# EndlessReform/fish-speech.rs

Hardware: AMD Instinct MI355X
Metric: codec tokens/sec (frames/s; 1 frame = 1 slow + 8 codebook tokens = 2048 PCM samples), Fish-1.5 batch=1 (higher is better)
Workload: dtype bf16

## Files before the change

### fish-speech.rs_amd/csrc/lm_engine.hip

```cpp
#include "lm_engine.h"

#include <algorithm>
#include <array>
#include <cmath>
#include <cstdlib>
#include <cstring>
#include <chrono>
#include <condition_variable>
#include <initializer_list>
#include <map>
#include <mutex>
#include <type_traits>
#include <vector>

#include <fcntl.h>
#include <sys/file.h>
#include <sys/stat.h>
#include <unistd.h>

#include "fs_common.h"
#include "fs_kv_pages.h"
#include "fs_prefill_plan.h"
#include "fs_synth.h"
#include "lm_kernels.h"
// ... 1573 lines not shown
            }
            launched += chunk;
            for (int b = 0; b < B_; ++b)
                if (slot_running(b)) {
                    sess_left_[b] -= chunk; sess_pos_[b] += chunk;
                    if (sess_left_[b] == 0 && !sess_.rows) {
                        static const int one = 1, zero = 0;
                        FS_HIP(hipMemcpyAsync(&state(b)->done, &one, sizeof(int), hipMemcpyHostToDevice, st_));
                        FS_HIP(hipMemcpyAsync(&state(b)->pos, &zero, sizeof(int), hipMemcpyHostToDevice, st_));
                        upload_row(b, st_, &sess_scratch_, 1);
                    }
                }
            FS_HIP(hipMemcpyAsync(sess_hs_.data(), state(0), sizeof(SeqState) * B_, hipMemcpyDeviceToHost, st_));
            tab_fetch_counts(hid_);
            tab_fetch_counts(sc_);
            FS_HIP(hipStreamSynchronize(st_));
            tab_take_counts(hid_);
            tab_take_counts(sc_);
            if (sess_.rows) rows_check_ctl(false);
            else check_rows_xchg();
        }
        FS_HIP(hipEventRecord(ev_[2], st_));
        FS_HIP(hipEventSynchronize(ev_[2]));
        float ms = 0;
        FS_HIP(hipEventElapsedTime(&ms, ev_[1], ev_[2]));
        stats_.decode_ms += ms;
        stats_.graph_launches += (uint64_t)launched;
        int act = 0;
        uint64_t frames = 0;
        for (int b = 0; b < B_; ++b) {
            if (slot_running(b) || slot_prefilling(b)) ++act;
            if (sess_left_[b] >= 0) frames += (uint64_t)sess_hs_[b].n_out;
        }
        stats_.frames = sess_released_frames_ + frames;
        if (n_active) *n_active = act;
    }
    void session_poll(int slot, uint32_t* codes_out, size_t cap, size_t* n_frames, int* done) override {
        use_device();
        require_live_slot(slot);
        const int C = a_.num_codebooks;
        const size_t nb = slot_prefilling(slot) ? 0 : (size_t)sess_hs_[slot].n_out;
        if (codes_out) {
            FS_REQUIRE(nb <= cap, "codes_out capacity too small for the generated frames");
            for (int c = 0; c < C; ++c)
                FS_HIP(hipMemcpyAsync(codes_out + (size_t)c * cap, d_out_.as<uint32_t>() + ((size_t)slot * C + c) * out_cap_, sizeof(uint32_t) * nb,
                                      hipMemcpyDeviceToHost, st_));
            FS_HIP(hipStreamSynchronize(st_));
        }
        if (n_frames) *n_frames = nb;
        if (done) *done = (!slot_prefilling(slot) && (sess_hs_[slot].done != 0 || sess_left_[slot] == 0)) ? 1 : 0;
    }
    void session_release(int slot) override {
        use_device();
        require_live_slot(slot);
        while (slot_prefilling(slot)) { flush_pending(); activate_pending(true); }
        sess_released_frames_ += (uint64_t)sess_hs_[slot].n_out;
        truncate(slot, 0);
        park_slot(slot, sess_.rows);
        tab_drop(hid_, slot);
        tab_drop(sc_, slot);
        sess_traced_[slot] = 0;
        sess_left_[slot] = kSlotFree;
    }
    void session_end() override {
        if (!sess_active_) return;
        use_device();
        if (!sess_flight_.empty()) (void)hipEventSynchronize(ev_pf_);
        std::string bad_book;
        try { pages_.check(); } catch (const std::exception& e) { bad_book = e.what(); }
        for (auto* q : {&sess_flight_, &sess_queue_})
            for (const PendingAdd& pa : *q) if (pa.tail >= 0) pages_.drop_hold(pa.tail);
        tab_end(hid_);
        tab_end(sc_);
        sess_flight_.clear(); sess_queue_.clear();
        pages_.end_session();
        std::fill(seq_len_.begin(), seq_len_.end(), 0);
        sess_prefixes_.clear();
        SampleCfg cfg = base_cfg();
        FS_HIP(hipMemcpyAsync(d_cfg_.p, &cfg, sizeof(cfg), hipMemcpyHostToDevice, st_));
        FS_HIP(hipStreamSynchronize(st_));
        sess_active_ = false;
        const bool rows = sess_.rows;
        sess_ = {};
        sess_released_frames_ = 0;
        if (rows) check_ctl({&d_rctl_s_, &d_rctl_f_}, nullptr, nullptr);
        if (sess_plock_.owns_lock()) sess_plock_.unlock();
        if (!bad_book.empty()) throw Error(bad_book);
    }

    void generate_batch_sequential(const uint32_t* prompts, const int* lens, int n, int max_new_tokens, const fs_sampling& s, uint64_t seed,
                                   uint32_t flags, uint32_t* codes_out, size_t cap, size_t* n_frames, uint8_t* is_audio) {
        if (legacy_) throw Error("generate_static_batch samples the slow token over the full vocabulary for Fish <= 1.4 (static_batch.rs:132-141); not implemented");
        const int C1 = a_.num_codebooks + 1;
        int Lmax = 0;
        for (int i = 0; i < n; ++i) { FS_REQUIRE(lens[i] >= 1, "empty prompt"); Lmax = std::max(Lmax, lens[i]); }
        fs_sampling sb = s;
        sb.repetition_penalty = 1.0f;
        size_t off = 0;
        std::vector<uint32_t> padded((size_t)C1 * Lmax);
        for (int i = 0; i < n; ++i) {
            left_pad(prompts + off, lens[i], Lmax, padded.data());
            off += (size_t)C1 * lens[i];
            clear_slow();
            batch_rows_ = n; batch_row_ = i;
            try {
                generate(padded.data(), Lmax, max_new_tokens, sb, seed, flags, codes_out + (size_t)i * a_.num_codebooks * cap, cap, &n_frames[i],
                         nullptr, nullptr, nullptr, 0, nullptr);
            } catch (...) { batch_rows_ = 0; batch_row_ = 0; throw; }
            batch_rows_ = 0; batch_row_ = 0;
            if (is_audio) {
                const SeqState* hs = reinterpret_cast<const SeqState*>(h_pin_);
                const bool first_not_audio = hs->frame == 1 && hs->cur[0] == t_.im_end_id;
                for (size_t f = 0; f < n_frames[i]; ++f) is_audio[(size_t)i * cap + f] = (f == 0 && first_not_audio) ? 0 : 1;
            }
        }
    }


    void generate_multi(const uint32_t* prompts, const int* lens, int n, const int* max_new_tokens, const fs_sampling* samplings,
                        const uint64_t* seeds, uint32_t flags, uint32_t* codes_out, size_t cap, size_t* n_frames) override {
        use_device();
        require_loaded();
        FS_REQUIRE(!sess_active_, "the handle is in session mode (fs_lm_session_end first)");
        FS_REQUIRE(n >= 1, "Must have at least one prompt");
        const int C = a_.num_codebooks, C1 = C + 1;
        std::vector<size_t> poff(n);
        {
            size_t off = 0;
            for (int i = 0; i < n; ++i) { FS_REQUIRE(lens[i] >= 1, "empty prompt"); FS_REQUIRE(max_new_tokens[i] >= 0, "negative max_new_tokens"); poff[i] = off; off += (size_t)C1 * lens[i]; }
        }
        bool rows_ok = rows_supported(n, samplings) && !(flags & FS_GEN_NO_PERSIST);
        const bool rows_sampled = samplings[0].temp != 0.0;
        std::unique_lock<PersistLock> plock;
        if (rows_ok) { plock = acquire_persist(device_); rows_ok = plock.owns_lock(); }
        if (!rows_ok) {
            if (plock.owns_lock()) plock.unlock();
            double pf = 0, dc = 0; uint64_t fr = 0, pt = 0, gl = 0;
            for (int i = 0; i < n; ++i) {
                clear_slow();
                generate(prompts + poff[i], lens[i], max_new_tokens[i], samplings[i], seeds[i], flags, codes_out + (size_t)i * C * cap, cap, &n_frames[i],
                         nullptr, nullptr, nullptr, 0, nullptr);
                pf += stats_.prefill_ms; dc += stats_.decode_ms; fr += stats_.frames; pt += stats_.prompt_tokens; gl += stats_.graph_launches;
            }
            stats_.prefill_ms = pf; stats_.decode_ms = dc; stats_.frames = fr; stats_.prompt_tokens = pt; stats_.graph_launches = gl;
            return;
        }
        const int R = n <= 2 ? 2 : (n <= 4 ? 4 : 8);
        ensure_rows(R);
        clear_slow();
        clear_fast();
        std::vector<long long> n_iter(n);
        long long max_iter = 0;
        for (int i = 0; i < n; ++i) {
            validate_tokens(prompts + poff[i], 0, 1, lens[i]);
            if (lens[i] > a_.max_seq_len) throw Error("prompt exceeds max_seq_len (dual_ar.rs:623-624)");
            n_iter[i] = iter_budget(max_new_tokens[i], lens[i]).n_iter;
            max_iter = std::max(max_iter, n_iter[i]);
            ensure_capacity(i, lens[i] + (int)n_iter[i] - 1);
        }
        std::vector<SampleCfg> cfgs(R);
        std::vector<int> budget(R, 0);
        for (int i = 0; i < R; ++i) {
            cfgs[i] = i < n ? make_cfg(samplings[i], flags) : base_cfg();
            if (i < n) budget[i] = (int)n_iter[i];
        }
        FS_HIP(hipMemcpyAsync(d_rcfg_.p, cfgs.data(), sizeof(SampleCfg) * R, hipMemcpyHostToDevice, st_));
        FS_HIP(hipMemcpyAsync(d_rbudget_.p, budget.data(), sizeof(int) * R, hipMemcpyHostToDevice, st_));
        float* nullp = nullptr;
        FS_HIP(hipMemcpyAsync(d_hid_slot_.p, &nullp, sizeof(nullp), hipMemcpyHostToDevice, st_));
        ensure_rows_capture(R);
        PersistFlagsGuard flags_guard{*this};
        stats_ = {};
        FS_HIP(hipEventRecord(ev_[0], st_));
        for (int i = 0; i < R; ++i) {
            SeqState ss = {};
            if (i >= n) { ss.done = 2; FS_HIP(hipMemcpyAsync(state(i), &ss, sizeof(ss), hipMemcpyHostToDevice, st_)); continue; }
            const int L = lens[i];
            ss.prompt_L = L;
            FS_HIP(hipMemcpyAsync(state(i), &ss, sizeof(ss), hipMemcpyHostToDevice, st_));
            FS_HIP(hipMemcpyAsync(main_.prompt.p, prompts + poff[i], sizeof(uint32_t) * C1 * L, hipMemcpyHostToDevice, st_));
            FS_HIP(hipMemcpyAsync(d_cfg_.p, &cfgs[i], sizeof(SampleCfg), hipMemcpyHostToDevice, st_));
            RngState rng;
            upload_rng(seeds[i], rng, d_rrng_.as<RngState>() + i, st_);
            launch_reppen_reset(rrp_.view(i), C, a_.codebook_size, st_);
            prefill_tokens(i, L - 1, false);
            LmKernels<WT>::embed(d_, tok_emb_, cb_emb_, C, a_.codebook_size, d_cfg_.as<SampleCfg>(), main_.prompt.as<uint32_t>(), state(i), x(i), st_);
            FS_HIP(hipStreamSynchronize(st_));
            seq_len_[i] = L - 1;
            stats_.prompt_tokens += (uint64_t)L;
        }
        use_persist_ = true; use_pslow_ = true; persist_sampled_ = rows_sampled;
        std::vector<SeqState> hs(R);
        auto all_done = [&]() {
            FS_HIP(hipMemcpyAsync(hs.data(), state(0), sizeof(SeqState) * R, hipMemcpyDeviceToHost, st_));
            FS_HIP(hipStreamSynchronize(st_));
            for (int i = 0; i < n; ++i) if (hs[i].done != 2) return false;
            return true;
        };
        int maxL = 0;
        for (int i = 0; i < n; ++i) maxL = std::max(maxL, lens[i]);
        const bool rows_fast = !getenv("FISHRT_ROWS_FAST_SINGLE");
        auto launch_frame = [&](long long it_) {
            set_bucket(maxL + (int)it_);
            RowsSlowArgs S = rows_slow_args(R);
            launch_rows_slow(S, R, st_);
            if (rows_fast) launch_rows_fast_groups(n, rows_sampled);
            else {
                static const int two = 2;
                for (int i = 0; i < n; ++i) {
                    if (it_ >= n_iter[i]) { if (it_ == n_iter[i]) FS_HIP(hipMemcpyAsync(&state(i)->done, &two, sizeof(int), hipMemcpyHostToDevice, st_)); continue; }
                    launch_fast_persist(persist_args(i), rows_sampled, st_);
                }
            }
        };
        launch_frame(0);
        FS_HIP(hipEventRecord(ev_[1], st_));
        long long it = 1;
        while (it < max_iter) {
            const long long end = std::min<long long>(max_iter, it + 32);
            for (; it < end; ++it) launch_frame(it);
            if (it < max_iter && all_done()) break;
        }
        if (!rows_fast) {
            static const int two = 2;
            for (int i = 0; i < n; ++i) FS_HIP(hipMemcpyAsync(&state(i)->done, &two, sizeof(int), hipMemcpyHostToDevice, st_));
        }
        FS_HIP(hipEventRecord(ev_[2], st_));
        FS_HIP(hipMemcpyAsync(hs.data(), state(0), sizeof(SeqState) * R, hipMemcpyDeviceToHost, st_));
        FS_HIP(hipStreamSynchronize(st_));
        use_persist_ = use_pslow_ = false;
        float ms01 = 0, ms12 = 0;
        FS_HIP(hipEventElapsedTime(&ms01, ev_[0], ev_[1]));
        FS_HIP(hipEventElapsedTime(&ms12, ev_[1], ev_[2]));
        stats_.prefill_ms = ms01; stats_.decode_ms = ms12; stats_.graph_launches = (uint64_t)it;
        stats_.kernels_per_frame = (uint64_t)(1 + (rows_fast ? (n + PR_FAST_ROWS - 1) / PR_FAST_ROWS : n));
        dump_rows_prof(R, it);
        rows_check_ctl(!rows_fast);
        stats_.frames = copy_out_rows(hs, n, codes_out, cap, n_frames);
    }

    bool rows_predicate(int n, const fs_sampling* ss, int ns, bool for_session, const char** why = nullptr) const {
        const char* w = nullptr;
        if (!(n >= 2 && n <= PR_MAX_ROWS && n <= B_)) w = "2 <= requests <= min(8, max_batch)";
        else if (!(loaded_ && pslow_ok_ && persist_ok_ && n_audio_ <= 2048)) w = "a loaded bf16 / fp8 handle with the Fish geometry on a 256-CU device";
        else if (getenv("FISHRT_NO_ROWS")) w = "FISHRT_NO_ROWS is set";
        else if (!rows_kv_span_ok(n <= 2 ? 2 : (n <= 4 ? 4 : 8))) w = "max_seq_len too long for the row kernels' attention slices at this row count";
        else if (for_session && legacy_) w = "row SESSIONS need the Fish 1.5 token layout (fs_lm_generate_multi serves Fish <= 1.4 handles)";
        else if (for_session && !(n == 2 || n == 4 || n == 8)) w = "row sessions need max_batch 2, 4 or 8";
        else {
            const bool sampled = ss[0].temp != 0.0;
            for (int i = 0; i < ns && !w; ++i) {
                if ((ss[i].temp != 0.0) != sampled) w = "every request greedy or every request sampled";
                else if (sampled && !fast_persist_samples((float)ss[i].temp, clamp_top_k(ss[i].top_k), a_.codebook_size)) w = "sampled requests with 0 < top_k <= 256";
            }
        }
        if (why) *why = w;
        return w == nullptr;
    }
    bool rows_supported(int n, const fs_sampling* samplings) override { return rows_predicate(n, samplings, n, false); }

  private:
    void use_device() { FS_HIP(hipSetDevice(device_)); }

    bool rows_kv_span_ok(int R) const {
        const int nslm = std::max(1, 16 / std::max(1, R));
        return ((a_.max_seq_len + nslm - 1) / nslm) / KV_PAGE + 2 <= 160;
    }
    void check_ctl(std::initializer_list<DevBuf*> bufs, const char* who, const char* bad_cfg_msg) {
        bool timeout = false, bad_cfg = false;
        for (DevBuf* cb : bufs) {
            if (!cb || !cb->p) continue;
            uint32_t ctl[4] = {0, 0, 0, 0};
            FS_HIP(hipMemcpy(ctl, cb->p, sizeof(ctl), hipMemcpyDeviceToHost));
            if (ctl[1] || ctl[2]) FS_HIP(hipMemset((uint32_t*)cb->p + 1, 0, 8));
            timeout |= ctl[1] != 0; bad_cfg |= ctl[2] != 0;
        }
        if (!who) return;
        if (timeout) {
            pslow_ok_ = persist_ok_ = false;
            throw Error(std::string(who) + ": a grid-wide wait timed out (are all 256 CUs available to this process?); "
                                           "the handle falls back to per-node launches for its next calls");
        }
        if (bad_cfg) throw Error(bad_cfg_msg);
    }
    void rows_check_ctl(bool include_b1_fast) {
        check_ctl({&d_rctl_s_, &d_rctl_f_, include_b1_fast ? &d_ctl_ : (DevBuf*)nullptr}, "request-row persistent kernels",
                  "request-row persistent kernels launched with a sampling configuration they were not built for");
    }
    void dump_persist_prof(int L) {
        if (!getenv("FISHRT_PERSIST_PROF")) return;
        unsigned long long pr[24];
        const double f = 0.01 / std::max<double>(1.0, (double)stats_.graph_launches - (double)L + 1);
        if (use_persist_) {
            FS_HIP(hipMemcpy(pr, d_ctl_.as<uint32_t>() + 16, sizeof(pr), hipMemcpyDeviceToHost));
            FS_HIP(hipMemset(d_ctl_.as<uint32_t>() + 16, 0, sizeof(pr)));
            fprintf(stderr, "persist prof (us/frame, workgroup 0; wait+work): preload %.1f  S1 %.1f+%.1f  S2 %.1f+%.1f  S3 %.1f+%.1f  S4 %.1f+%.1f  head %.1f+%.1f  decision %.1f+%.1f  tail %.1f | S3 split: gemv+reduce %.1f barrier %.1f epilogue %.1f\n",
                    pr[0] * f, pr[9] * f, pr[1] * f, pr[10] * f, pr[2] * f, pr[11] * f, pr[3] * f, pr[12] * f, pr[4] * f, pr[13] * f, pr[5] * f, pr[14] * f, pr[6] * f, pr[7] * f, pr[8] * f, pr[15] * f, pr[3] * f);
            fprintf(stderr, "persist boundaries (us/frame, workgroup 0): slow kernel's finish -> fast kernel's entry %.2f (%llu frames)  entry -> first stage timer (state, slow-token decision) %.2f  last timer -> finish %.2f\n",
                    pr[20] ? pr[17] * 0.01 / (double)pr[20] : 0.0, pr[20], pr[18] * f, pr[19] * f);
        }
        if (use_pslow_) {
            FS_HIP(hipMemcpy(pr, d_sctl_.as<uint32_t>() + 16, sizeof(pr), hipMemcpyDeviceToHost));
            FS_HIP(hipMemset(d_sctl_.as<uint32_t>() + 16, 0, sizeof(pr)));
            fprintf(stderr, "slow persist prof (us/frame, workgroup %d; wait+work): S1 %.1f+%.1f  S2 %.1f+%.1f  S3 %.1f+%.1f  S4 %.1f+%.1f  S5 %.1f+%.1f  head %.1f+%.1f\n",
                    getenv("FISHRT_PERSIST_PROF_WG") ? atoi(getenv("FISHRT_PERSIST_PROF_WG")) : 0, pr[9] * f, pr[1] * f, pr[10] * f, pr[2] * f, pr[11] * f, pr[3] * f,
                    pr[12] * f, pr[4] * f, pr[13] * f, pr[5] * f, pr[14] * f, pr[6] * f);
            fprintf(stderr, "slow persist boundaries (us/frame): fast kernel's finish -> slow kernel's entry %.2f (%llu frames)  entry -> first stage timer (state, first loads) %.2f  last timer -> finish %.2f\n",
                    pr[20] ? pr[17] * 0.01 / (double)pr[20] : 0.0, pr[20], pr[18] * f, pr[19] * f);
        }
    }
    void dump_rows_prof(int R, long long frames) {
        if (!getenv("FISHRT_PERSIST_PROF")) return;
        unsigned long long pr[16];
        const double f = 0.01 / std::max<double>(1.0, (double)frames);
        FS_HIP(hipMemcpy(pr, d_rctl_s_.as<uint32_t>() + 16, sizeof(pr), hipMemcpyDeviceToHost));
        FS_HIP(hipMemset(d_rctl_s_.as<uint32_t>() + 16, 0, sizeof(pr)));
        fprintf(stderr, "rows slow prof R=%d (us/frame, workgroup 0): S1 %.1f  S2 %.1f  S3 sweep %.1f + %.1f  S4 sweep %.1f gemm %.1f barrier %.1f publish %.1f  S5 sweep+gemm %.1f barrier %.1f publish %.1f  head %.1f\n",
                R, pr[1] * f, pr[2] * f, pr[8] * f, pr[3] * f, pr[9] * f, pr[10] * f, pr[11] * f, pr[4] * f, pr[12] * f, pr[13] * f, pr[5] * f, pr[6] * f);
        FS_HIP(hipMemcpy(pr, d_rctl_f_.as<uint32_t>() + 16, sizeof(pr), hipMemcpyDeviceToHost));
        FS_HIP(hipMemset(d_rctl_f_.as<uint32_t>() + 16, 0, sizeof(pr)));
        fprintf(stderr, "rows fast prof (us/frame summed over the fast launches, workgroup 0; wait+work): preload %.1f  S1 %.1f+%.1f  S2 %.1f+%.1f  S3 %.1f+%.1f  S4 %.1f+%.1f  head %.1f+%.1f  decision %.1f+%.1f (rows' logits -> argmax / draw %.1f, pick -> next input %.1f)  tail %.1f\n",
                pr[0] * f, pr[9] * f, pr[1] * f, pr[10] * f, pr[2] * f, pr[11] * f, (pr[3] + pr[8]) * f, pr[12] * f, pr[4] * f, pr[13] * f, pr[5] * f, pr[14] * f, (pr[6] + pr[15]) * f, pr[15] * f, pr[6] * f, pr[7] * f);
    }
    void upload_rng(uint64_t seed, RngState& host, RngState* dst, hipStream_t st) {
        host = RngState{};
        seed_from_u64(seed, host.key);
        FS_HIP(hipMemcpyAsync(dst, &host, sizeof(host), hipMemcpyHostToDevice, st));
    }
    void left_pad(const uint32_t* prompt, int L, int Lmax, uint32_t* out) const {
        const int C1 = a_.num_codebooks + 1, pad = Lmax - L;
        for (int r = 0; r < C1; ++r) {
            for (int j = 0; j < pad; ++j) out[(size_t)r * Lmax + j] = r == 0 ? t_.im_end_id : 0u;
            std::memcpy(&out[(size_t)r * Lmax + pad], prompt + (size_t)r * L, sizeof(uint32_t) * L);
        }
    }
    uint64_t copy_out_rows(const std::vector<SeqState>& hs, int n, uint32_t* codes_out, size_t cap, size_t* n_frames) {
        const int C = a_.num_codebooks;
        std::vector<uint32_t> tmp((size_t)n * C * out_cap_);
        FS_HIP(hipMemcpy(tmp.data(), d_out_.p, sizeof(uint32_t) * tmp.size(), hipMemcpyDeviceToHost));
        uint64_t total = 0;
        for (int i = 0; i < n; ++i) {
            const size_t nb = (size_t)hs[i].n_out;
            FS_REQUIRE(nb <= cap, "codes_out capacity too small for the generated frames");
            for (int c = 0; c < C; ++c)
                std::memcpy(codes_out + ((size_t)i * C + c) * cap, tmp.data() + ((size_t)i * C + c) * out_cap_, sizeof(uint32_t) * nb);
            n_frames[i] = nb;
            total += nb;
            seq_len_[i] = hs[i].pos;
        }
        return total;
    }
    void launch_rows_fast_groups(int top, bool sampled) {
        for (int r0 = 0; r0 < top; r0 += PR_FAST_ROWS) {
            const int left = std::min(PR_FAST_ROWS, top - r0), Rf = left >= 3 ? 4 : left;
            launch_rows_fast(rows_fast_args(r0, Rf), Rf, sampled, st_);
        }
    }
    struct PersistFlagsGuard {
        LM& lm;
        ~PersistFlagsGuard() { lm.use_persist_ = lm.use_pslow_ = false; }
    };
    void require_loaded() { FS_REQUIRE(loaded_, "weights not loaded: call fs_lm_load_safetensors or fs_lm_load_synthetic first"); }

    static int clamp_top_k(uint64_t top_k) { return (int)std::min<uint64_t>(top_k, 1u << 30); }
    SampleCfg make_cfg(const fs_sampling& s, uint32_t flags) const {
        SampleCfg c = base_cfg();
        c.temp = (float)s.temp; c.top_p = (float)s.top_p; c.top_p64 = s.top_p;
        c.top_k = clamp_top_k(s.top_k);
        c.rep_pen = s.repetition_penalty; c.ignore_eos = (flags & FS_GEN_IGNORE_EOS) ? 1 : 0;
        return c;
    }
    struct Budget { long long n_iter; bool clamped; };
    Budget iter_budget(long long max_new, long long L_total, long long n_cached = 0) const {
        Budget b{1 + std::max<long long>(0, max_new - L_total + 1), false};
        const long long room = (long long)a_.max_seq_len - (n_cached + L_total) + 1;
        if (b.n_iter > room) { b.n_iter = room; b.clamped = true; }
        FS_REQUIRE(b.n_iter <= out_cap_, "generation longer than the output staging buffer");
        return b;
    }
    SampleCfg base_cfg() const {
        SampleCfg c = {};
        c.temp = 0.f; c.top_p = 1.f; c.top_k = 0; c.rep_pen = 1.f; c.ignore_eos = 0;
        c.im_end_id = t_.im_end_id;
        c.audio_base = legacy_ ? t_.im_end_id : t_.semantic_start_id - 1;
        c.sem_lo = t_.semantic_start_id;
        c.sem_hi = t_.has_semantic_end ? t_.semantic_end_id : t_.semantic_start_id;
        c.legacy = legacy_ ? 1 : 0;
        c.pad_id = t_.pad_id;
        return c;
    }

    void validate_tokens(const uint32_t* toks, size_t, int B, int L) {
        const int C1 = a_.num_codebooks + 1;
        for (int b = 0; b < B; ++b)
            for (int r = 0; r < C1; ++r)
                for (int l = 0; l < L; ++l) {
                    const uint32_t v = toks[((size_t)b * C1 + r) * L + l];
                    if (r == 0) { if (v >= (uint32_t)a_.vocab_size) throw Error("token id out of vocabulary (index_select out of range)"); }
                    else if (v >= (uint32_t)a_.codebook_size) throw Error("codebook id out of range (index_select out of range)");
                }
    }

    void plan_tensors() {
        size_t off = 0;
        auto align = [&](size_t v) { return (v + 255) & ~(size_t)255; };
        auto mat = [&](const std::string& name, int64_t rows, int64_t cols, int mul, int roff, std::pair<size_t, size_t> at) {
            tensors_.push_back({name, rows, cols, false, false, at.first, at.second, mul, roff, 0.f, 0.02});
        };
        auto emb = [&](const std::string& name, int64_t rows, int64_t cols) {
            size_t at = off;
            off = align(off + (size_t)rows * cols * sizeof(KT));
            tensors_.push_back({name, rows, cols, false, true, at, 0, 1, 0, 0.f, 0.02});
            return at;
        };
        auto slab = [&](int64_t rows, int64_t cols) {
            std::pair<size_t, size_t> at{off, 0};
            off = align(off + (size_t)rows * cols * sizeof(WT));
            if (kFp8) { at.second = off; off = align(off + (size_t)rows * sizeof(float)); }
            return at;
        };
        auto vec = [&](const std::string& name, int64_t n) {
            size_t at = off;
            off = align(off + (size_t)n * sizeof(float));
            tensors_.push_back({name, 1, n, true, false, at, 0, 1, 0, 1.0f, 0.1});
            return at;
        };
        const int64_t D = a_.dim, I = a_.intermediate_size, V = a_.vocab_size;
        const int64_t QKV = (int64_t)(a_.n_head + 2 * a_.n_local_heads) * a_.head_dim;
        o_tok_emb_ = emb("embeddings.weight", V, D);
        o_cb_emb_ = emb("codebook_embeddings.weight", (int64_t)a_.codebook_size * a_.num_codebooks, D);
        auto blocks = [&](int n, const std::string& pre, std::vector<std::array<size_t, 10>>& offs) {
            for (int l = 0; l < n; ++l) {
                const std::string p = pre + std::to_string(l) + ".";
                std::array<size_t, 10> o;
                auto s0 = slab(QKV, D); mat(p + "attention.wqkv.weight", QKV, D, 1, 0, s0);
                auto s1 = slab(D, D); mat(p + "attention.wo.weight", D, D, 1, 0, s1);
                auto s2 = slab(2 * I, D);
                mat(p + "feed_forward.w1.weight", I, D, 2, 0, s2);
                mat(p + "feed_forward.w3.weight", I, D, 2, 1, s2);
                auto s3 = slab(D, I); mat(p + "feed_forward.w2.weight", D, I, 1, 0, s3);
                o[0] = s0.first; o[1] = s1.first; o[2] = s2.first; o[3] = s3.first;
                o[4] = vec(p + "ffn_norm.weight", D);
                o[5] = vec(p + "attention_norm.weight", D);
                o[6] = s0.second; o[7] = s1.second; o[8] = s2.second; o[9] = s3.second;
                offs.push_back(o);
            }
        };
        blocks(a_.n_layer, "layers.", o_slow_);
        o_norm_ = vec("norm.weight", D);
        if (a_.tie_word_embeddings && !kFp8) o_out_ = {o_tok_emb_, 0};
        else { o_out_ = slab(V, D); mat(a_.tie_word_embeddings ? "embeddings.weight" : "output.weight", V, D, 1, 0, o_out_); }
        o_fast_emb_ = emb("fast_embeddings.weight", a_.codebook_size, D);
        blocks(a_.n_fast_layer, "fast_layers.", o_fast_);
        o_fast_norm_ = vec("fast_norm.weight", D);
        o_fast_out_ = slab(a_.codebook_size, D); mat("fast_output.weight", a_.codebook_size, D, 1, 0, o_fast_out_);
        arena_bytes_ = off;
    }

    void alloc_runtime() {
        arena_.alloc(arena_bytes_);
        uint8_t* base = arena_.as<uint8_t>();
        auto lw = [&](const std::array<size_t, 10>& o) {
            LayerW w;
            w.wqkv = base + o[0]; w.wo = base + o[1]; w.w13 = base + o[2]; w.w2 = base + o[3];
            w.ffn_norm = (const float*)(base + o[4]); w.attn_norm = (const float*)(base + o[5]);
            if (kFp8) {
                w.s_qkv = (const float*)(base + o[6]); w.s_o = (const float*)(base + o[7]);
                w.s_13 = (const float*)(base + o[8]); w.s_2 = (const float*)(base + o[9]);
            }
            return w;
        };
        for (auto& o : o_slow_) slow_.push_back(lw(o));
        for (auto& o : o_fast_) { fast_.push_back(lw(o)); fast_.back().cache_resident = getenv("FISHRT_FAST_NT") == nullptr; }
        tok_emb_ = base + o_tok_emb_; cb_emb_ = base + o_cb_emb_; fast_emb_ = base + o_fast_emb_;
        out_w_ = base + o_out_.first; fast_out_w_ = base + o_fast_out_.first;
        if (kFp8) { out_s_ = (const float*)(base + o_out_.second); fast_out_s_ = (const float*)(base + o_fast_out_.second); }
        norm_w_ = (const float*)(base + o_norm_); fast_norm_w_ = (const float*)(base + o_fast_norm_);
        const int half = a_.head_dim / 2, n_elem = a_.dim / a_.n_head;
        std::vector<float> ct((size_t)a_.max_seq_len * half), sn((size_t)a_.max_seq_len * half), theta(half);
        for (int j = 0; j < half; ++j) theta[j] = 1.f / std::pow(a_.rope_base, (float)(2 * j) / (float)n_elem);
        for (int p = 0; p < a_.max_seq_len; ++p)
            for (int j = 0; j < half; ++j) {
                const float ang = (float)p * theta[j];
                ct[(size_t)p * half + j] = std::cos(ang);
                sn[(size_t)p * half + j] = std::sin(ang);
            }
        d_cos_.alloc(ct.size() * 4); d_sin_.alloc(sn.size() * 4);
        FS_HIP(hipMemcpy(d_cos_.p, ct.data(), ct.size() * 4, hipMemcpyHostToDevice));
        FS_HIP(hipMemcpy(d_sin_.p, sn.data(), sn.size() * 4, hipMemcpyHostToDevice));
        n_chunks_ = (a_.max_seq_len + AttnKernels<WT>::chunk() - 1) / AttnKernels<WT>::chunk();
        FS_REQUIRE(n_chunks_ <= 128, "max_seq_len too large for the attention chunking (128 chunks)");
        max_pages_ = std::max((a_.max_seq_len + KV_PAGE - 1) / KV_PAGE, n_chunks_ * AttnKernels<WT>::chunk() / KV_PAGE);
        n_pages_ = max_pages_ * B_;
        page_elems_ = (size_t)a_.n_local_heads * KV_PAGE * a_.head_dim;
        kv_pool_.alloc((size_t)a_.n_layer * 2 * n_pages_ * page_elems_ * sizeof(KT));
        FS_HIP(hipMemset(kv_pool_.p, 0, kv_pool_.n));
        d_page_table_.alloc(sizeof(int) * (size_t)std::max(2 * B_ + 1, PR_MAX_ROWS) * max_pages_);
        FS_HIP(hipMemset(d_page_table_.p, 0, d_page_table_.n));
        pages_.init(n_pages_, B_, KV_PAGE, a_.max_seq_len);
        seq_len_.assign(B_, 0);
        fast_len_.assign(B_, 0);
        fast_pool_.alloc((size_t)std::max(1, a_.n_fast_layer) * 2 * B_ * page_elems_ * sizeof(KT));
        FS_HIP(hipMemset(fast_pool_.p, 0, fast_pool_.n));
        d_zero_table_.alloc(sizeof(int) * 4);
        FS_HIP(hipMemset(d_zero_table_.p, 0, d_zero_table_.n));
        d_x_.alloc(sizeof(float) * (size_t)std::max(B_, PR_MAX_ROWS) * a_.dim);
        d_xf_.alloc(sizeof(float) * (size_t)std::max(B_, PR_MAX_ROWS) * a_.dim);
        FS_HIP(hipMemset(d_x_.p, 0, d_x_.n));
        d_q_.alloc(sizeof(float) * a_.dim);
        d_part_.alloc(sizeof(float) * (size_t)a_.n_head * n_chunks_ * (a_.head_dim + 2));
        FS_HIP(hipMemset(d_part_.p, 0, d_part_.n));
        d_act_.alloc(sizeof(float) * a_.intermediate_size);
        d_logits_slow_.alloc(sizeof(float) * a_.vocab_size);
        d_logits_fast_.alloc(sizeof(float) * a_.codebook_size);
        d_hid_slot_.alloc(sizeof(float*));
        FS_HIP(hipMemset(d_hid_slot_.p, 0, sizeof(float*)));
        d_state_.alloc(sizeof(SeqState) * (std::max(B_, PR_MAX_ROWS) + 1));
        FS_HIP(hipMemset(d_state_.p, 0, d_state_.n));
        d_cfg_.alloc(sizeof(SampleCfg));
        SampleCfg c = base_cfg();
        FS_HIP(hipMemcpy(d_cfg_.p, &c, sizeof(c), hipMemcpyHostToDevice));
        d_rng_.alloc(sizeof(RngState));
        main_.prompt.alloc(sizeof(uint32_t) * (size_t)(a_.num_codebooks + 1) * a_.max_seq_len);
        out_cap_ = a_.max_seq_len + 8;
        d_out_.alloc(sizeof(uint32_t) * (size_t)B_ * a_.num_codebooks * out_cap_);
        rp_.alloc(1, a_.num_codebooks, a_.codebook_size);
        FS_HIP(hipHostMalloc(&h_pin_, 4096, hipHostMallocDefault));
    }

    const void* slow_head_w() {
        if (!legacy_ && !generic_) return (const uint8_t*)out_w_ + (size_t)t_.im_end_id * a_.dim * sizeof(WT);
        if (!d_legacy_head_.p) d_legacy_head_.alloc(gathered_head_bytes() + sizeof(float) * n_audio_ + 256);
        return d_legacy_head_.p;
    }
    size_t gathered_head_bytes() const { return ((sizeof(WT) * (size_t)n_audio_ * a_.dim) + 15) & ~(size_t)15; }
    const float* slow_head_s() {
        if (!kFp8) return nullptr;
        if (!legacy_ && !generic_) return out_s_ + t_.im_end_id;
        slow_head_w();
        return (const float*)(d_legacy_head_.as<uint8_t>() + gathered_head_bytes());
    }
    void refresh_legacy_head() {
        if (generic_) {
            const size_t row = sizeof(WT) * (size_t)a_.dim;
            uint8_t* dst = (uint8_t*)const_cast<void*>(slow_head_w());
            FS_HIP(hipMemcpyAsync(dst, (const uint8_t*)out_w_ + t_.im_end_id * row, row, hipMemcpyDeviceToDevice, st_));
            FS_HIP(hipMemcpyAsync(dst + row, (const uint8_t*)out_w_ + t_.semantic_start_id * row, row * (n_audio_ - 1), hipMemcpyDeviceToDevice, st_));
            if (kFp8) {
                float* ds = const_cast<float*>(slow_head_s());
                FS_HIP(hipMemcpyAsync(ds, out_s_ + t_.im_end_id, sizeof(float), hipMemcpyDeviceToDevice, st_));
                FS_HIP(hipMemcpyAsync(ds + 1, out_s_ + t_.semantic_start_id, sizeof(float) * (n_audio_ - 1), hipMemcpyDeviceToDevice, st_));
            }
            FS_HIP(hipStreamSynchronize(st_));
            return;
        }
        if (!legacy_) return;
        launch_gather_rows<WT>(out_w_, a_.dim, t_.pad_id, t_.im_end_id, const_cast<void*>(slow_head_w()), st_);
        if (kFp8) launch_gather_rows<float>(out_s_, 1, t_.pad_id, t_.im_end_id, const_cast<float*>(slow_head_s()), st_);
        FS_HIP(hipStreamSynchronize(st_));
    }
    SeqState* state(int b) { return d_state_.as<SeqState>() + b; }
    float* x(int b) { return d_x_.as<float>() + (size_t)b * a_.dim; }
    float* xf(int b) { return d_xf_.as<float>() + (size_t)b * a_.dim; }
    KVView slow_kv(int layer, int b) {
        KVView v;
        KT* base = kv_pool_.as<KT>() + (size_t)layer * 2 * n_pages_ * page_elems_;
        v.k = base; v.v = base + (size_t)n_pages_ * page_elems_;
        v.page_table = d_page_table_.as<int>() + (size_t)b * max_pages_;
        return v;
    }
    KVView fast_kv(int layer, int b) {
        KVView v;
        KT* base = fast_pool_.as<KT>() + ((size_t)layer * 2 * B_) * page_elems_;
        v.k = base + (size_t)b * page_elems_;
        v.v = base + ((size_t)B_ + b) * page_elems_;
        v.page_table = d_zero_table_.as<int>();
        return v;
    }

    void ensure_capacity(int b, int n_tokens) {
        if (!pages_.grow(b, n_tokens)) return;
        upload_row(b, st_, pages_.of(b));
        FS_HIP(hipStreamSynchronize(st_));
    }
    void truncate(int b, int pos) {
        pages_.truncate(b, pos);
        seq_len_[b] = pos;
    }
    void upload_row(int row, hipStream_t st, const int* ids, size_t n) {
        FS_HIP(hipMemcpyAsync(d_page_table_.as<int>() + (size_t)row * max_pages_, ids, sizeof(int) * n, hipMemcpyHostToDevice, st));
    }
    void upload_row(int row, hipStream_t st, const std::vector<int>& ids) { upload_row(row, st, ids.data(), ids.size()); }

    void prefill_tokens(int b, int n, bool use_graph) {
        if (n <= 0) return;
        if (RowKernels<WT>::has_mfma_prefill() && n > 1 && a_.dim % 128 == 0 && a_.intermediate_size % 128 == 0) {
            ensure_prefill_buffers();
            const int M = launch_seq_pass(main_, state(b), b, seq_len_[b], n);
            FS_HIP(hipMemcpyAsync(x(b), main_.x.as<float>() + (size_t)(M - 1) * a_.dim, sizeof(float) * a_.dim, hipMemcpyDeviceToDevice, st_));
            return;
        }
        for (int l = 0; l < n; ++l) {
            set_bucket(seq_len_[b] + l + 1);
            if (use_graph && b == 0) { use_graphs_for_bucket(); FS_HIP(hipGraphLaunch(g_step_, st_)); continue; }
            LmKernels<WT>::embed(d_, tok_emb_, cb_emb_, a_.num_codebooks, a_.codebook_size, d_cfg_.as<SampleCfg>(),
                                 main_.prompt.as<uint32_t>(), state(b), x(b), st_);
            enqueue_slow_layers(b);
            launch_advance(state(b), st_);
        }
    }
    int launch_seq_pass(PrefillLane& ln, SeqState* st, int kv_row, int start, int n) {
        RowsCtx c = ln.ctx(st, 1, 0);
        int M = 0;
        for (int done = 0; done < n; done += M) {
            M = std::min(a_.head_dim == 64 ? kRowsCap : kPartRows, n - done);
            c.nc_launch = chunk_bucket(start + done + M);
            RowKernels<WT>::prefill_embed(d_, tok_emb_, cb_emb_, a_.num_codebooks, a_.codebook_size, d_cfg_.as<SampleCfg>(),
                                         ln.prompt.as<uint32_t>(), st, M, ln.x.as<float>(), ln.st);
            for (int l = 0; l < a_.n_layer; ++l) RowKernels<WT>::rows_layer(d_, M, c, slow_[l], slow_kv(l, kv_row), l == 0, ln.st);
            RowKernels<WT>::rows_finish(d_, M, c, nullptr, ln.st);
            launch_advance_n(st, M, ln.st);
        }
        return M;
    }
    void launch_group_pass(PrefillLane& ln, const uint32_t* prompts, int S, int Lp, size_t pstride, SeqState* st, int kv_row,
                           const SeqState* seq_states, int nc_launch) {
        RowsCtx c = ln.ctx(st, 1, max_pages_);
        c.seq_rows = Lp;
        c.nc_launch = nc_launch;
        c.seq_states = seq_states;
        const int M = S * Lp;
        RowKernels<WT>::prefill_embed(d_, tok_emb_, cb_emb_, a_.num_codebooks, a_.codebook_size, d_cfg_.as<SampleCfg>(), prompts, st, M,
                                     ln.x.as<float>(), ln.st, Lp, pstride);
        for (int l = 0; l < a_.n_layer; ++l) RowKernels<WT>::rows_layer(d_, M, c, slow_[l], slow_kv(l, kv_row), l == 0, ln.st);
    }
    void ensure_prefill_buffers() {
        if (main_.x.p) return;
        const int I = a_.intermediate_size;
        down_split_ = I % 1024 == 0 ? I / 1024 : (I % 256 == 0 ? I / 256 : I / 128);
        main_.ensure(a_, down_split_, n_chunks_, d_cos_.as<float>(), d_sin_.as<float>());
    }
    void check_rows_xchg() {
        if (!d_epoch_.p) return;
        uint32_t e[2] = {0, 0};
        FS_HIP(hipMemcpy(e, d_epoch_.p, sizeof(e), hipMemcpyDeviceToHost));
        if (e[1] != 0) {
            const uint32_t z = 0;
            FS_HIP(hipMemcpy(d_epoch_.as<uint32_t>() + 1, &z, sizeof(z), hipMemcpyHostToDevice));
            fold_off_ = true;
            drop_batch_graphs();
            throw Error("static-batch decode: " + std::to_string(e[1]) + " split-K exchange waits timed out (a down projection's blocks were not co-resident); "
                        "this handle falls back to the slab path for its next calls");
        }
    }
    void ensure_batch_buffers() {
        if (d_xfrows_.p) return;
        ld_slow_ = ((n_audio_ + 63) / 64) * 64;
        d_xfrows_.alloc(sizeof(float) * kRows * a_.dim);
        d_lrows_.alloc(sizeof(float) * kRows * ld_slow_);
        d_lfast_.alloc(sizeof(float) * kRows * a_.codebook_size);
        std::vector<SeqState> fs(8);
        for (int i = 0; i < 8; ++i) { fs[i] = SeqState{}; fs[i].pos = i; }
        d_fast_state_.alloc(sizeof(SeqState) * 8);
        FS_HIP(hipMemcpy(d_fast_state_.p, fs.data(), sizeof(SeqState) * 8, hipMemcpyHostToDevice));
        std::vector<int> tb(B_);
        for (int i = 0; i < B_; ++i) tb[i] = i;
        d_rwords_.alloc(sizeof(uint32_t) * 16 * kRows);
        d_xchg_.alloc(rows_xchg_bytes(a_.dim));
        FS_HIP(hipMemset(d_xchg_.p, 0, d_xchg_.n));
        d_epoch_.alloc(sizeof(uint32_t) * 2);
        const uint32_t e0[2] = {1u, 0u};
        FS_HIP(hipMemcpy(d_epoch_.p, e0, sizeof(e0), hipMemcpyHostToDevice));
        d_fast_table_.alloc(sizeof(int) * B_);
        FS_HIP(hipMemcpy(d_fast_table_.p, tb.data(), sizeof(int) * B_, hipMemcpyHostToDevice));
        hid_.dev.alloc(sizeof(HidSlot) * B_);
        FS_HIP(hipMemset(hid_.dev.p, 0, hid_.dev.n));
        sc_.dev.alloc(sizeof(ScoreSlot) * B_);
        FS_HIP(hipMemset(sc_.dev.p, 0, sc_.dev.n));
    }
    void enqueue_batch_frame(int B) {
        const int C = a_.num_codebooks;
        RowsCtx cs = main_.ctx(state(0), sess_active_ ? -1 : 0, max_pages_);
        cs.nc_launch = nc_launch_;
        cs.xchg = d_xchg_.p; cs.epoch = d_epoch_.as<uint32_t>();
        const bool fold = !fold_off_ && RowKernels<WT>::rows_fold_ok(d_, B, cs) && a_.n_layer <= 64 && a_.n_fast_layer <= 8 && C <= 32;
        cs.fold = fold;
        for (int l = 0; l < a_.n_layer; ++l, cs.node_id = (uint32_t)l)
            RowKernels<WT>::rows_layer(d_, B, cs, slow_[l], slow_kv(l, 0), l == 0, st_, fold ? (l + 1 < a_.n_layer ? slow_[l + 1].attn_norm : norm_w_) : nullptr);
        if (!fold) RowKernels<WT>::rows_finish(d_, B, cs, norm_w_, st_);
        RowKernels<WT>::rows_head(d_, B, cs, slow_head_w(), slow_head_s(), n_audio_, d_lrows_.as<float>(), ld_slow_, st_, fold);
        if (sess_active_) launch_hidden_rows(hid_.dev.as<HidSlot>(), state(0), cs.X, a_.dim, B, st_);
        const bool slots = sess_.slots;
        const uint32_t* words = rows_par_ ? d_rwords_.as<uint32_t>() : nullptr;
        if (rows_par_) SampleKernels<WT>::rows_rng_words(d_rng_.as<RngState>(), B, C + 1, state(0), d_rwords_.as<uint32_t>(), st_);
        const bool capt = cap_frames_ > 0 && d_rcap_.p && d_rcap_.n >= sizeof(float) * (size_t)B * cap_frames_ * 9 * 2048;
        if (capt) launch_cap_rows_logits(d_lrows_.as<float>(), ld_slow_, n_audio_, state(0), d_cfg_.as<SampleCfg>(), B, d_rcap_.as<float>(), cap_frames_, 0, st_);
        const float* prep_g = fold && a_.dim <= 1024 ? fast_[0].attn_norm : nullptr;
        const bool score = slots && sess_.score;
        const bool trace = score && sess_.trace;
        float* stash = trace ? d_trace_.as<float>() : nullptr;
        const int alts = score ? sess_.alts : 0;
        if (score) launch_score_slots(sc_.dev.as<ScoreSlot>(), state(0), d_scfg_.as<SampleCfg>(), d_lrows_.as<float>(), ld_slow_, n_audio_, 0, C, B, st_, stash, alts);
        if (slots)
            SampleKernels<WT>::sample_slow_slots(d_, d_lrows_.as<float>(), ld_slow_, n_audio_, d_scfg_.as<SampleCfg>(), d_srng_.as<SlotRng>(), B, state(0),
                                                 cs.X, d_xfrows_.as<float>(), st_, prep_g, cs.A, fold ? d_epoch_.as<uint32_t>() : nullptr,
                                                 capt ? d_rcap_.as<float>() : nullptr, cap_frames_, sess_.wide);
        else
        SampleKernels<WT>::sample_slow_rows(d_, d_lrows_.as<float>(), ld_slow_, n_audio_, d_cfg_.as<SampleCfg>(), d_rng_.as<RngState>(), B,
                                            C + 1, state(0), cs.X, d_xfrows_.as<float>(), st_, words, prep_g, cs.A, fold ? d_epoch_.as<uint32_t>() : nullptr);
        const bool qkv0_on = fold && d_qkv0_.p && !getenv("FISHRT_ROWS_NO_QKV0") && a_.codebook_size == 1024;
        auto fast_ctx = [&](int cbi) {
            RowsCtx cf = cs;
            cf.X = d_xfrows_.as<float>();
            cf.state = d_fast_state_.as<SeqState>() + cbi;
            cf.pos_step = 0;
            cf.pt_stride = 1;
            cf.nc_launch = 1;
            cf.small_attn = a_.num_codebooks <= 8;
            cf.identity_pages = true;
            cf.attn_t1 = cbi == 0;
            if (qkv0_on && AttnKernels<WT>::rows_qkv0_ok(d_, cf)) { cf.qkv0_tbl = d_qkv0_.as<float>(); cf.row_states = state(0); cf.code_slot = cbi; }
            return cf;
        };
        RowsCtx cf = fast_ctx(0);
        cf.first_prepped = prep_g != nullptr;
        for (int cbi = 0; cbi < C; ++cbi) {
            for (int l = 0; l < a_.n_fast_layer; ++l) {
                KVView kv;
                KT* base = fast_pool_.as<KT>() + ((size_t)l * 2 * B_) * page_elems_;
                kv.k = base; kv.v = base + (size_t)B_ * page_elems_; kv.page_table = d_fast_table_.as<int>();
                cf.node_id = 64u + (uint32_t)cbi * 8u + (uint32_t)l;
                RowKernels<WT>::rows_layer(d_, B, cf, fast_[l], kv, l == 0, st_, fold ? (l + 1 < a_.n_fast_layer ? fast_[l + 1].attn_norm : fast_norm_w_) : nullptr);
            }
            if (!fold) RowKernels<WT>::rows_finish(d_, B, cf, fast_norm_w_, st_);
            RowKernels<WT>::rows_head(d_, B, cf, fast_out_w_, kFp8 ? fast_out_s_ : nullptr, a_.codebook_size, d_lfast_.as<float>(), a_.codebook_size, st_, fold);
            if (capt) launch_cap_rows_logits(d_lfast_.as<float>(), a_.codebook_size, a_.codebook_size, state(0), d_cfg_.as<SampleCfg>(), B, d_rcap_.as<float>(),
                                             cap_frames_, 1 + cbi, st_);
            RowsCtx nf = fast_ctx(cbi + 1);
            const float* prep_f = nf.qkv0_tbl ? nullptr : prep_g;
            nf.first_prepped = prep_f != nullptr;
            if (score) launch_score_slots(sc_.dev.as<ScoreSlot>(), state(0), d_scfg_.as<SampleCfg>(), d_lfast_.as<float>(), a_.codebook_size, a_.codebook_size,
                                          1 + cbi, C, B, st_, stash, alts);
            if (slots) {
                RepPenState rp0 = srp_.view(0);
                SampleKernels<WT>::sample_fast_slots(d_, d_lfast_.as<float>(), cbi, C, a_.codebook_size, d_scfg_.as<SampleCfg>(), d_srng_.as<SlotRng>(), rp0,
                                                     B, state(0), fast_emb_, d_xfrows_.as<float>(), tok_emb_, cb_emb_, cs.X, d_out_.as<uint32_t>(), out_cap_,
                                                     st_, prep_f, cs.A, sess_.wide);
            } else
            SampleKernels<WT>::sample_fast_rows(d_, d_lfast_.as<float>(), cbi, C, a_.codebook_size, d_cfg_.as<SampleCfg>(),
                                                d_rng_.as<RngState>(), B, state(0), fast_emb_, d_xfrows_.as<float>(), tok_emb_, cb_emb_,
                                                cs.X, d_out_.as<uint32_t>(), out_cap_, st_, words, prep_f, cs.A);
            cf = nf;
        }
        if (trace) launch_trace_commit(sc_.dev.as<ScoreSlot>(), state(0), d_scfg_.as<SampleCfg>(), stash, n_audio_, a_.codebook_size, C, B, st_, alts);
        if (capt) launch_cap_rows_picks(state(0), d_cfg_.as<SampleCfg>(), B, d_rcap_.as<float>(), cap_frames_, C, st_);
    }
    void ensure_rows_capture(int B) {
        if (!cap_frames_) return;
        FS_REQUIRE((size_t)B * cap_frames_ <= 4096, "decision capture on the row path: rows x frames limited to 4096 (302 MB)");
        d_rcap_.alloc(sizeof(float) * (size_t)B * cap_frames_ * 9 * 2048);
        FS_HIP(hipMemsetAsync(d_rcap_.p, 0, d_rcap_.n, st_));
    }
    void drop_batch_graphs() {
        for (auto& kv : batch_graphs_) if (kv.second) (void)hipGraphExecDestroy(kv.second);
        batch_graphs_.clear();
    }
    void destroy_graphs() {
        for (auto& kv : graphs_)
            for (hipGraphExec_t g : {kv.second.first, kv.second.second}) if (g) (void)hipGraphExecDestroy(g);
        graphs_.clear();
        for (auto& kv : multi_graphs_) if (kv.second) (void)hipGraphExecDestroy(kv.second);
        multi_graphs_.clear();
        g_frame_ = g_step_ = nullptr;
        drop_batch_graphs();
    }
    hipGraphExec_t batch_graph(int B) {
        const long long key = (sess_active_ ? 1 << 24 : 0) + (rows_par_ ? 1 << 25 : 0) + (sess_.slots ? 1 << 26 : 0) + (sess_.slots && sess_.wide ? 1 << 27 : 0) +
                              (sess_.slots && sess_.score ? 1 << 28 : 0) + (sess_.slots && sess_.score && sess_.trace ? 1 << 29 : 0) + B * 1024 + nc_launch_ +
                              ((long long)(sess_.slots && sess_.score ? sess_.alts : 0) << 32);
        auto it = batch_graphs_.find(key);
        if (it != batch_graphs_.end()) return it->second;
        {
            RowsCtx cs = main_.ctx(state(0), 0, max_pages_);
            cs.xchg = d_xchg_.p; cs.epoch = d_epoch_.as<uint32_t>();
            (void)RowKernels<WT>::rows_fold_ok(d_, B, cs);
        }
        hipGraph_t g = nullptr;
        hipGraphExec_t ge = nullptr;
        FS_HIP(hipStreamBeginCapture(st_, hipStreamCaptureModeThreadLocal));
        enqueue_batch_frame(B);
        FS_HIP(hipStreamEndCapture(st_, &g));
        FS_HIP(hipGraphInstantiate(&ge, g, nullptr, nullptr, 0));
        FS_HIP(hipGraphDestroy(g));
        batch_graphs_[key] = ge;
        return ge;
    }

    static constexpr int kNapsFast[6] = {16, 16, 16, 16, 16, 16}, kNapsSlow[6] = {20, 16, 6, 36, 36, 12};
    static constexpr int kNapsFastSampled[6] = {12, 16, 12, 20, 12, 16}, kNapsSlowFp8[6] = {20, 4, 28, 24, 24, 0};
    static constexpr bool kSlowStreamNt = true, kSlowStreamNtFp8 = true;
    static void set_naps(int (&naps)[6], const char* env, const int (&dflt)[6]) {
        for (int i = 0; i < 6; ++i) naps[i] = dflt[i];
        if (const char* v = getenv(env)) {
            int i = 0;
            for (const char* p = v; *p && i < 6; ++i) { naps[i] = atoi(p); while (*p && *p != ',') ++p; if (*p == ',') ++p; }
        }
    }
    void pack_persist() {
        persist_ok_ = false;
        if (d_qkv0_.p) { destroy_graphs(); d_qkv0_.free(); }
        if constexpr (std::is_same<WT, bf16_t>::value || std::is_same<WT, fp8_t>::value) {
            constexpr bool FP8 = std::is_same<WT, fp8_t>::value;
            if (getenv("FISHRT_NO_PERSIST")) return;
            if (!fast_persist_supported(d_, a_.n_fast_layer, a_.num_codebooks, a_.codebook_size)) return;
            hipDeviceProp_t prop;
            FS_HIP(hipGetDeviceProperties(&prop, device_));
            if (prop.multiProcessorCount < PF_BLOCKS) return;
            if (!d_pack_.p) {
                d_pack_.alloc(fast_persist_pack_bytes());
                d_edges_.alloc(fast_persist_edge_bytes());
                FS_HIP(hipMemset(d_edges_.p, 0, d_edges_.n));
                d_ctl_.alloc(320);
                FS_HIP(hipMemset(d_ctl_.p, 0, d_ctl_.n));
                if (FP8) d_fscl_.alloc(sizeof(float) * (size_t)PF_BLOCKS * PF_SCL);
            }
            launch_fast_persist_pack(fast_.data(), fast_out_w_, d_pack_.p, st_, FP8, fast_out_s_, d_fscl_.as<float>());
            if (!getenv("FISHRT_FAST_NO_QKV0")) {
                d_qkv0_.alloc(fast_persist_qkv0_bytes());
                launch_fast_persist_qkv0_table(d_pack_.p, FP8 ? d_fscl_.as<float>() : nullptr, fast_[0].attn_norm, fast_emb_, d_.eps, d_qkv0_.as<float>(), st_);
            }
            FS_HIP(hipStreamSynchronize(st_));
            persist_ok_ = true;
            pslow_ok_ = false;
            if (getenv("FISHRT_NO_PERSIST_SLOW") || n_audio_ > 8 * PF_BLOCKS) return;
            if (const char* c = getenv("FISHRT_SLOW_STREAM"))
                FS_REQUIRE(strcmp(c, "default") == 0 || strcmp(c, "nt") == 0, "FISHRT_SLOW_STREAM must be 'default' or 'nt'");
            if (!d_spack_.p) {
                d_spack_.alloc(slow_persist_pack_bytes(a_.n_layer, FP8));
                d_hpack_.alloc((size_t)PF_BLOCKS * PS_HEAD_IMAGE);
                if (FP8) d_sscl_.alloc(sizeof(float) * slow_persist_scale_floats(a_.n_layer));
                d_snorms_.alloc(sizeof(float) * (size_t)(2 * a_.n_layer + 1) * a_.dim);
                d_sedges_.alloc(slow_persist_edge_bytes());
                FS_HIP(hipMemset(d_sedges_.p, 0, d_sedges_.n));
                d_sctl_.alloc(320);
                FS_HIP(hipMemset(d_sctl_.p, 0, d_sctl_.n));
            }
            std::vector<const float*> np;
            for (int l = 0; l < a_.n_layer; ++l) { np.push_back(slow_[l].attn_norm); np.push_back(slow_[l].ffn_norm); }
            np.push_back(norm_w_);
            if (FP8) launch_slow_persist_pack_fp8(slow_.data(), a_.n_layer, slow_head_w(), slow_head_s(), n_audio_, np.data(), d_spack_.p, d_hpack_.p,
                                                  d_sscl_.as<float>(), d_snorms_.as<float>(), st_);
            else launch_slow_persist_pack(slow_.data(), a_.n_layer, slow_head_w(), n_audio_, np.data(), d_spack_.p, d_hpack_.p, d_snorms_.as<float>(), st_);
            FS_HIP(hipStreamSynchronize(st_));
            pslow_ok_ = true;
        }
    }
    SlowPersistArgs pslow_args() {
        SlowPersistArgs A = {};
        A.wpack = d_spack_.p; A.hpack = d_hpack_.p; A.norms = d_snorms_.as<float>();
        A.scales = d_sscl_.p ? d_sscl_.as<float>() : nullptr;
        A.hscales = d_sscl_.p ? d_sscl_.as<float>() + (size_t)a_.n_layer * PF_BLOCKS * 48 : nullptr;
        A.n_layer = a_.n_layer; A.n_head_rows = n_audio_;
        A.cos_t = d_cos_.as<float>(); A.sin_t = d_sin_.as<float>(); A.eps = d_.eps;
        A.x = x(0); A.logits = d_logits_slow_.as<float>(); A.state = state(0);
        A.kv_pool = kv_pool_.p; A.layer_half = (size_t)n_pages_ * page_elems_;
        A.page_table = d_page_table_.as<int>();
        A.n_sl = std::min(nc_launch_, nc_launch_ > 32 ? 16 : 8);
        if (const char* c = getenv("FISHRT_NSL_MAX")) A.n_sl = std::max(1, std::min(A.n_sl, atoi(c)));
        if (const char* c = getenv("FISHRT_NSL_MIN")) A.n_sl = std::min(16, std::max(A.n_sl, atoi(c)));
        while (A.n_sl & (A.n_sl - 1)) A.n_sl &= A.n_sl - 1;
        A.edges = d_sedges_.as<unsigned long long>();
        A.ctl = d_sctl_.as<uint32_t>();
        A.prof = getenv("FISHRT_PERSIST_PROF") ? reinterpret_cast<unsigned long long*>(d_sctl_.as<uint32_t>() + 16) : nullptr;
        A.peer_stamps = (A.prof && d_ctl_.p) ? reinterpret_cast<const unsigned long long*>(d_ctl_.as<uint32_t>() + 16) + 16 : nullptr;
        set_naps(A.naps, "FISHRT_NAPS_SLOW", kFp8 ? kNapsSlowFp8 : kNapsSlow);
        A.prof_wg = getenv("FISHRT_PERSIST_PROF_WG") ? atoi(getenv("FISHRT_PERSIST_PROF_WG")) : 0;
        A.l2_touch = (getenv("FISHRT_SLOW_EARLY") ? atoi(getenv("FISHRT_SLOW_EARLY")) : (kFp8 ? 1 : 9)) & 15;
        bool stream_nt = kFp8 ? kSlowStreamNtFp8 : kSlowStreamNt;
        if (const char* c = getenv("FISHRT_SLOW_STREAM")) stream_nt = strcmp(c, "nt") == 0;
        if (stream_nt) A.l2_touch |= PS_STREAM_NT;
        return A;
    }
    bool fold_slow_sampler() const { return use_persist_ && n_audio_ <= 2048; }
    FastPersistArgs persist_args() {
        FastPersistArgs A = {};
        A.wpack = d_pack_.p;
        A.scales = d_fscl_.p ? d_fscl_.as<float>() : nullptr;
        for (int l = 0; l < PF_LAYERS; ++l) { A.norms[2 * l] = fast_[l].attn_norm; A.norms[2 * l + 1] = fast_[l].ffn_norm; }
        A.norms[2 * PF_LAYERS] = fast_norm_w_;
        A.fast_emb = fast_emb_; A.tok_emb = tok_emb_; A.cb_emb = cb_emb_;
        A.qkv0_tbl = d_qkv0_.p ? d_qkv0_.as<float>() : nullptr;
        A.cos_t = d_cos_.as<float>(); A.sin_t = d_sin_.as<float>();
        A.eps = d_.eps;
        const bool fold = fold_slow_sampler();
        A.xf = fold ? x(0) : xf(0); A.x = x(0);
        A.slow_logits = fold ? d_logits_slow_.as<float>() : nullptr; A.n_slow = n_audio_; A.hid_slot = d_hid_slot_.as<float*>();
        A.cap = d_cap_.as<float>(); A.cap_frames = cap_frames_;
        A.state = state(0); A.cfg = d_cfg_.as<SampleCfg>(); A.rp = rp_.view(0); A.rng = d_rng_.as<RngState>();
        A.out_codes = d_out_.as<uint32_t>(); A.out_cap = out_cap_;
        A.edges = d_edges_.as<unsigned long long>();
        A.ctl = d_ctl_.as<uint32_t>();
        A.prof = getenv("FISHRT_PERSIST_PROF") ? reinterpret_cast<unsigned long long*>(d_ctl_.as<uint32_t>() + 16) : nullptr;
        A.peer_stamps = (A.prof && d_sctl_.p) ? reinterpret_cast<const unsigned long long*>(d_sctl_.as<uint32_t>() + 16) + 16 : nullptr;
        set_naps(A.naps, "FISHRT_NAPS_FAST", persist_sampled_ ? kNapsFastSampled : kNapsFast);
        return A;
    }


    void ensure_rows(int R) {
        if constexpr (std::is_same<WT, bf16_t>::value || kFp8) {
            if (!d_rimg_.p) {
                d_rimg_.alloc(slow_persist_pack_bytes(a_.n_layer, false));
                d_rhimg_.alloc((size_t)PF_BLOCKS * PS_HEAD_IMAGE);
                if constexpr (kFp8) launch_rows_pack_fp8(slow_.data(), a_.n_layer, slow_head_w(), n_audio_, d_rimg_.p, d_rhimg_.p, st_);
                else launch_rows_pack(slow_.data(), a_.n_layer, slow_head_w(), n_audio_, d_rimg_.p, d_rhimg_.p, st_);
                if constexpr (!kFp8) {
                    const size_t n1 = (size_t)a_.n_layer * PF_BLOCKS * 48 + (size_t)PF_BLOCKS * 8 + (size_t)PF_BLOCKS * PF_SCL;
                    std::vector<float> ones(n1, 1.0f);
                    d_rones_.alloc(n1 * sizeof(float));
                    FS_HIP(hipMemcpyAsync(d_rones_.p, ones.data(), n1 * sizeof(float), hipMemcpyHostToDevice, st_));
                    FS_HIP(hipStreamSynchronize(st_));
                }
                d_rpairs_.alloc((size_t)PF_BLOCKS * 40 * PF_THREADS * 4);
                launch_rows_pack_rowpairs(d_pack_.p, d_rpairs_.p, st_);
                d_redges_s_.alloc(rows_slow_edge_bytes(PR_MAX_ROWS));
                FS_HIP(hipMemsetAsync(d_redges_s_.p, 0, d_redges_s_.n, st_));
                d_redges_f_.alloc(rows_fast_edge_bytes(PR_FAST_ROWS));
                FS_HIP(hipMemsetAsync(d_redges_f_.p, 0, d_redges_f_.n, st_));
                d_rctl_s_.alloc(256); d_rctl_f_.alloc(256);
                FS_HIP(hipMemsetAsync(d_rctl_s_.p, 0, 256, st_));
                FS_HIP(hipMemsetAsync(d_rctl_f_.p, 0, 256, st_));
                d_rlogits_.alloc(sizeof(float) * PR_MAX_ROWS * PR_LD);
                d_rcfg_.alloc(sizeof(SampleCfg) * PR_MAX_ROWS);
                d_rrng_.alloc(sizeof(RngState) * PR_MAX_ROWS);
                d_rbudget_.alloc(sizeof(int) * PR_MAX_ROWS);
                rrp_.alloc(PR_MAX_ROWS, a_.num_codebooks, a_.codebook_size);
                FS_HIP(hipStreamSynchronize(st_));
            }
            (void)R;
        } else {
            throw Error("request rows need a bf16 or fp8 handle");
        }
    }
    static constexpr int kNapsRowsSlow[6] = {28, 4, 8, 40, 24, 28}, kNapsRowsFast[6] = {20, 16, 16, 16, 20, 20};
    RowsSlowArgs rows_slow_args(int R) {
        RowsSlowArgs A = {};
        A.wimg = d_rimg_.p; A.himg = d_rhimg_.p; A.norms = d_snorms_.as<float>();
        const float* sc0 = kFp8 ? d_sscl_.as<float>() : d_rones_.as<float>();
        A.scales = sc0;
        A.hscales = sc0 + (size_t)a_.n_layer * PF_BLOCKS * 48;
        A.n_layer = a_.n_layer; A.n_head_rows = n_audio_;
        A.cos_t = d_cos_.as<float>(); A.sin_t = d_sin_.as<float>(); A.eps = d_.eps;
        A.x = x(0); A.logits = d_rlogits_.as<float>(); A.state = state(0);
        A.kv_pool = kv_pool_.p; A.layer_half = (size_t)n_pages_ * page_elems_;
        A.page_table = d_page_table_.as<int>(); A.pt_stride = max_pages_;
        A.n_sl = std::max(1, std::min(nc_launch_, 16 / R));
        if (const char* c = getenv("FISHRT_ROWS_NSL_MAX")) A.n_sl = std::max(1, std::min(A.n_sl, atoi(c)));
        A.edges = d_redges_s_.as<unsigned long long>();
        A.ctl = d_rctl_s_.as<uint32_t>();
        A.prof = getenv("FISHRT_PERSIST_PROF") ? reinterpret_cast<unsigned long long*>(d_rctl_s_.as<uint32_t>() + 16) : nullptr;
        set_naps(A.naps, "FISHRT_NAPS_ROWS_SLOW", kNapsRowsSlow);
        return A;
    }
    RowsFastArgs rows_fast_args(int r0, int Rf) {
        RowsFastArgs A = {};
        (void)Rf;
        A.wpack = d_pack_.p; A.rowpairs = d_rpairs_.as<uint32_t>();
        A.scales = kFp8 ? d_fscl_.as<float>() : d_rones_.as<float>() + (size_t)a_.n_layer * PF_BLOCKS * 48 + (size_t)PF_BLOCKS * 8;
        for (int l = 0; l < PF_LAYERS; ++l) { A.norms[2 * l] = fast_[l].attn_norm; A.norms[2 * l + 1] = fast_[l].ffn_norm; }
        A.norms[2 * PF_LAYERS] = fast_norm_w_;
        A.fast_emb = fast_emb_; A.tok_emb = tok_emb_; A.cb_emb = cb_emb_;
        A.qkv0_tbl = (d_qkv0_.p && !getenv("FISHRT_ROWS_FAST_NO_QKV0")) ? d_qkv0_.as<float>() : nullptr;
        A.cos_t = d_cos_.as<float>(); A.sin_t = d_sin_.as<float>(); A.eps = d_.eps;
        A.xf = x(r0); A.x = x(r0);
        A.slow_logits = d_rlogits_.as<float>() + (size_t)r0 * PR_LD; A.n_slow = n_audio_;
        A.cap = cap_frames_ ? d_rcap_.as<float>() + (size_t)r0 * cap_frames_ * 9 * 2048 : nullptr; A.cap_frames = cap_frames_;
        A.state = state(r0); A.cfg = d_rcfg_.as<SampleCfg>() + r0; A.budget = d_rbudget_.as<int>() + r0; A.rng = d_rrng_.as<RngState>() + r0;
        const RepPenState rp = rrp_.view(r0);
        A.rp_mask = rp.mask; A.rp_ring = rp.ring; A.rp_meta = rp.ring_meta;
        A.out_codes = d_out_.as<uint32_t>() + (size_t)r0 * a_.num_codebooks * out_cap_; A.out_cap = out_cap_;
        A.edges = d_redges_f_.as<unsigned long long>();
        A.ctl = d_rctl_f_.as<uint32_t>();
        A.prof = getenv("FISHRT_PERSIST_PROF") ? reinterpret_cast<unsigned long long*>(d_rctl_f_.as<uint32_t>() + 16) : nullptr;
        set_naps(A.naps, "FISHRT_NAPS_ROWS_FAST", kNapsRowsFast);
        A.nap_draw = getenv("FISHRT_NAP_ROWS_DRAW") ? atoi(getenv("FISHRT_NAP_ROWS_DRAW")) : 16;
        return A;
    }
    FastPersistArgs persist_args(int i) {
        FastPersistArgs A = persist_args();
        A.xf = x(i); A.x = x(i);
        A.slow_logits = d_rlogits_.as<float>() + (size_t)i * PR_LD;
        A.cap = cap_frames_ ? d_rcap_.as<float>() + (size_t)i * cap_frames_ * 9 * 2048 : nullptr;
        A.state = state(i); A.cfg = d_rcfg_.as<SampleCfg>() + i; A.rp = rrp_.view(i); A.rng = d_rrng_.as<RngState>() + i;
        A.out_codes = d_out_.as<uint32_t>() + (size_t)i * a_.num_codebooks * out_cap_;
        return A;
    }

    void enqueue_slow_layers(int b) {
        for (int l = 0; l < a_.n_layer; ++l) {
            const LayerW& w = slow_[l];
            KVView kv = slow_kv(l, b);
            LmKernels<WT>::qkv(d_, x(b), w, d_cos_.as<float>(), d_sin_.as<float>(), state(b), 0, 0, d_q_.as<float>(), kv, st_);
            AttnKernels<WT>::decode(d_, d_q_.as<float>(), kv, state(b), d_part_.as<float>(), n_chunks_, nc_launch_, st_);
            LmKernels<WT>::wo(d_, d_part_.as<float>(), n_chunks_, nc_launch_, state(b), nullptr, kv, 0, w, x(b), st_);
            LmKernels<WT>::ffn_up(d_, x(b), w, d_act_.as<float>(), st_);
            LmKernels<WT>::ffn_down(d_, d_act_.as<float>(), w, x(b), st_);
        }
    }
    void enqueue_fast_layers(int b, int kv_pos, int rope_pos) {
        for (int l = 0; l < a_.n_fast_layer; ++l) {
            const LayerW& w = fast_[l];
            KVView kv = fast_kv(l, b);
            LmKernels<WT>::qkv(d_, xf(b), w, d_cos_.as<float>(), d_sin_.as<float>(), nullptr, kv_pos, rope_pos, d_q_.as<float>(), kv, st_);
            LmKernels<WT>::wo(d_, nullptr, 0, 0, nullptr, d_q_.as<float>(), kv, kv_pos + 1, w, xf(b), st_);
            LmKernels<WT>::ffn_up(d_, xf(b), w, d_act_.as<float>(), st_);
            LmKernels<WT>::ffn_down(d_, d_act_.as<float>(), w, xf(b), st_);
        }
    }

    int chunk_bucket(int T) const {
        const int need = (T + AttnKernels<WT>::chunk() - 1) / AttnKernels<WT>::chunk();
        int b = 1;
        while (b < need) b <<= 1;
        return std::min(b, n_chunks_);
    }
    void set_bucket(int T) { nc_launch_ = chunk_bucket(T); }
    void use_graphs_for_bucket() {
        const int key = nc_launch_ * 8 + (use_persist_ && persist_sampled_ ? 4 : 0) + (use_persist_ ? 2 : 0) + (use_pslow_ ? 1 : 0);
        auto it = graphs_.find(key);
        if (it == graphs_.end()) {
            g_frame_ = nullptr; g_step_ = nullptr;
            build_graphs();
            graphs_[key] = {g_frame_, g_step_};
        } else {
            g_frame_ = it->second.first; g_step_ = it->second.second;
        }
    }
    void build_graphs() {
        if (g_frame_) return;
        FS_REQUIRE(a_.num_codebooks <= 8, "the fused fast-decoder attention holds at most 8 positions");
        const int C = a_.num_codebooks;
        hipGraph_t g = nullptr;
        FS_HIP(hipStreamBeginCapture(st_, hipStreamCaptureModeThreadLocal));
        LmKernels<WT>::embed(d_, tok_emb_, cb_emb_, C, a_.codebook_size, d_cfg_.as<SampleCfg>(), main_.prompt.as<uint32_t>(), state(0), x(0), st_);
        enqueue_slow_layers(0);
        launch_advance(state(0), st_);
        FS_HIP(hipStreamEndCapture(st_, &g));
        FS_HIP(hipGraphInstantiate(&g_step_, g, nullptr, nullptr, 0));
        FS_HIP(hipGraphDestroy(g));
        FS_HIP(hipStreamBeginCapture(st_, hipStreamCaptureModeThreadLocal));
        if (use_pslow_) launch_slow_persist(pslow_args(), st_);
        else {
        enqueue_slow_layers(0);
        LmKernels<WT>::head(d_, x(0), norm_w_, slow_head_w(), slow_head_s(), n_audio_, d_logits_slow_.as<float>(), st_);
        }
        if (!fold_slow_sampler())
            SampleKernels<WT>::sample_slow(d_, d_logits_slow_.as<float>(), n_audio_, d_cfg_.as<SampleCfg>(), d_rng_.as<RngState>(), state(0),
                                           x(0), xf(0), st_, d_hid_slot_.as<float*>());
        if (use_persist_) launch_fast_persist(persist_args(), persist_sampled_, st_);
        else
        for (int cbi = 0; cbi < C; ++cbi) {
            enqueue_fast_layers(0, cbi, cbi);
            LmKernels<WT>::head(d_, xf(0), fast_norm_w_, fast_out_w_, fast_out_s_, a_.codebook_size, d_logits_fast_.as<float>(), st_);
            SampleKernels<WT>::sample_fast(d_, d_logits_fast_.as<float>(), cbi, C, a_.codebook_size, d_cfg_.as<SampleCfg>(),
                                           d_rng_.as<RngState>(), rp_.view(0), state(0), fast_emb_, xf(0), tok_emb_, cb_emb_, x(0),
                                           d_out_.as<uint32_t>(), out_cap_, st_);
        }
        FS_HIP(hipStreamEndCapture(st_, &g));
        FS_HIP(hipGraphInstantiate(&g_frame_, g, nullptr, nullptr, 0));
        FS_HIP(hipGraphDestroy(g));
    }

    fs_model_args a_;
    fs_token_cfg t_;
    int device_, B_;
    ModelDims d_;
    int n_audio_ = 0;
    bool generic_ = false;
    bool legacy_ = false;
    DevBuf d_legacy_head_;
    hipStream_t st_ = nullptr;
    bool loaded_ = false;
    std::vector<TensorDesc> tensors_;
    size_t arena_bytes_ = 0, o_tok_emb_ = 0, o_cb_emb_ = 0, o_fast_emb_ = 0, o_norm_ = 0, o_fast_norm_ = 0;
    std::pair<size_t, size_t> o_out_ = {0, 0}, o_fast_out_ = {0, 0};
    std::vector<std::array<size_t, 10>> o_slow_, o_fast_;
    DevBuf arena_;
    std::vector<LayerW> slow_, fast_;
    const void *tok_emb_ = nullptr, *cb_emb_ = nullptr, *fast_emb_ = nullptr, *out_w_ = nullptr, *fast_out_w_ = nullptr;
    const float *norm_w_ = nullptr, *fast_norm_w_ = nullptr, *out_s_ = nullptr, *fast_out_s_ = nullptr;
    DevBuf d_cos_, d_sin_;
    int max_pages_ = 0, n_pages_ = 0, out_cap_ = 0, n_chunks_ = 0, nc_launch_ = 1;
    std::map<int, std::pair<hipGraphExec_t, hipGraphExec_t>> graphs_;
    std::map<int, hipGraphExec_t> multi_graphs_;
    static int frames_per_graph() {
        static const int v = [] { const char* e = getenv("FISHRT_FRAMES_PER_GRAPH"); const int n = e ? atoi(e) : 8; return n < 0 ? 1 : (n > 32 ? 32 : n); }();
        return v;
    }
    hipGraphExec_t multi_frame_graph() {
        const int key = nc_launch_ * 8 + (persist_sampled_ ? 4 : 0);
        auto it = multi_graphs_.find(key);
        if (it != multi_graphs_.end()) return it->second;
        hipGraph_t g = nullptr;
        hipGraphExec_t ge = nullptr;
        FS_HIP(hipStreamBeginCapture(st_, hipStreamCaptureModeThreadLocal));
        for (int f = 0; f < frames_per_graph(); ++f) {
            launch_slow_persist(pslow_args(), st_);
            launch_fast_persist(persist_args(), persist_sampled_, st_);
        }
        FS_HIP(hipStreamEndCapture(st_, &g));
        FS_HIP(hipGraphInstantiate(&ge, g, nullptr, nullptr, 0));
        FS_HIP(hipGraphDestroy(g));
        multi_graphs_[key] = ge;
        return ge;
    }
    size_t page_elems_ = 0;
    DevBuf kv_pool_, fast_pool_, d_page_table_, d_zero_table_;
    KvPages pages_;
    std::vector<int> seq_len_, fast_len_;
    DevBuf d_x_, d_xf_, d_q_, d_part_, d_act_, d_logits_slow_, d_logits_fast_, d_state_, d_cfg_, d_rng_, d_out_;
    RepPenBufs rp_, srp_, rrp_;
    DevBuf d_pack_, d_edges_, d_ctl_, d_qkv0_;
    DevBuf d_fscl_, d_sscl_;
    DevBuf d_cap_;
    int cap_frames_ = 0;
    DevBuf d_hidden_, d_hid_slot_;
    bool persist_ok_ = false, use_persist_ = false, pslow_ok_ = false, use_pslow_ = false, persist_sampled_ = false;
    int batch_rows_ = 0, batch_row_ = 0;
    bool sess_active_ = false;
    struct SessMode {
        bool rows = false;
        bool sampled = false;
        int R = 0;
        bool slots = false;
        bool wide = false;
        bool score = false;
        bool trace = false;
        int alts = 0;
    } sess_{};
    SampleCfg sess_cfg_ = {};
    DevBuf d_scfg_, d_srng_;
    int sess_adds_ = 0, sess_budget_tmp_ = 0;
    uint64_t sess_seed_ = 0;
    std::unique_lock<PersistLock> sess_plock_;
    std::vector<int> sess_left_, sess_pos_;
    std::vector<int> sess_L_;
    std::vector<SeqState> sess_hs_;
    int sess_scratch_ = 0;
    uint64_t sess_released_frames_ = 0;
    std::vector<SessPrefix> sess_prefixes_;
    std::vector<SeqState> sess_stage_pos0_;
    std::vector<int> sess_stage_copy_;
    DevBuf d2_seqpos_, d2_copy_;
    DevBuf d_promo_pair_;
    hipEvent_t ev_pft_[2] = {nullptr, nullptr};
    bool sess_timed_ = false;
    int64_t sess_count_[4] = {0, 0, 0, 0};
    double sess_pf_ms_ = 0.0;
    std::vector<uint32_t> sess_stage_prompts_;
    std::vector<int> sess_stage_rows_;
    std::vector<PendingAdd> sess_queue_, sess_flight_;
    DevBuf d_kvb_, d_kvb_pages_, d_fp_;
    std::vector<int> sess_stage_imp_pages_;
    bool fp_valid_ = false;
    uint64_t fp_ = 0;
    SlotTab<HidSlot> hid_;
    SlotTab<ScoreSlot> sc_;
    std::vector<char> sess_traced_;
    DevBuf d_trace_;
    SeqState sess_stage_ = {};
    hipStream_t st_pf_ = nullptr;
    hipEvent_t ev_pf_ = nullptr;
    PrefillLane join_{st_pf_};
    DevBuf d_spack_, d_hpack_, d_snorms_, d_sedges_, d_sctl_;
    PrefillLane main_{st_};
    DevBuf d_bprompt_;
    DevBuf d_xfrows_, d_lrows_, d_lfast_, d_fast_state_, d_fast_table_, d_rwords_;
    DevBuf d_xchg_, d_epoch_;
    bool rows_par_ = false;
    int ld_slow_ = 0, down_split_ = 4;
    bool fold_off_ = false;
    std::map<long long, hipGraphExec_t> batch_graphs_;
    DevBuf d_rimg_, d_rhimg_, d_redges_s_, d_redges_f_, d_rctl_s_, d_rctl_f_, d_rlogits_, d_rcfg_, d_rrng_, d_rbudget_;
    DevBuf d_rcap_, d_rpairs_, d_rones_;
    void* h_pin_ = nullptr;
    hipGraphExec_t g_frame_ = nullptr, g_step_ = nullptr;
    hipEvent_t ev_[3] = {nullptr, nullptr, nullptr};
    hipEvent_t ev_batch_[2] = {nullptr, nullptr};
    fs_gen_stats stats_ = {};
};

void fp8_quantize_rows(int device, const float* w, int64_t rows, int64_t cols, uint8_t* q_out, float* scales_out) {
    FS_REQUIRE(rows >= 1 && cols >= 1 && rows < (1ll << 31), "bad matrix shape");
    FS_HIP(hipSetDevice(device));
    DevBuf src, q, sc;
    src.alloc((size_t)rows * cols * 4); q.alloc((size_t)rows * cols); sc.alloc((size_t)rows * 4);
    FS_HIP(hipMemcpy(src.p, w, (size_t)rows * cols * 4, hipMemcpyHostToDevice));
    launch_quant_rows_fp8(q.as<uint8_t>(), sc.as<float>(), src.as<float>(), rows, cols, 1, 0, nullptr);
    FS_HIP(hipDeviceSynchronize());
    FS_HIP(hipMemcpy(q_out, q.p, (size_t)rows * cols, hipMemcpyDeviceToHost));
    FS_HIP(hipMemcpy(scales_out, sc.p, (size_t)rows * 4, hipMemcpyDeviceToHost));
}
void fp8_decode_table(int device, float* out) {
    FS_HIP(hipSetDevice(device));
    DevBuf t;
    t.alloc(16 * 256 * 4);
    launch_fp8_decode_table(t.as<float>(), nullptr);
    FS_HIP(hipDeviceSynchronize());
    FS_HIP(hipMemcpy(out, t.p, 16 * 256 * 4, hipMemcpyDeviceToHost));
}

LMBase* make_lm(const fs_model_args& a, const fs_token_cfg& t, int device, fs_dtype dtype, int max_batch) {
    if (dtype == FS_BF16) return new LM<bf16_t>(a, t, device, max_batch);
    if (dtype == FS_F32) return new LM<float>(a, t, device, max_batch);
    if (dtype == FS_FP8) return new LM<fp8_t>(a, t, device, max_batch);
    throw Error("unknown dtype");
}

}
```

### fish-speech.rs_amd/csrc/lm_persist.h

```cpp
#pragma once
#include <hip/hip_runtime.h>

#include <cstdint>

#include "lm_kernels.h"

namespace fs {

constexpr int PF_BLOCKS = 256;
constexpr int PF_THREADS = 512;
constexpr int PF_REPL = 8;
constexpr int PF_EDGE_CAP = 4096;
constexpr int PF_RING = 4;
constexpr int PF_LAYERS = 4;
constexpr int PF_REG_DW = PF_LAYERS * (5 + 4 + 32) + 4;
constexpr int PF_REG_CHUNKS = PF_REG_DW / 4;
constexpr int PF_ROW_CHUNKS = (PF_LAYERS * 9 + 4) / 4;
constexpr int PF_LDS_CHUNKS = PF_LAYERS * 4;
constexpr int PF_CHUNKS = PF_REG_CHUNKS + PF_LDS_CHUNKS;
constexpr int PF_SCL = 200;

struct FastPersistArgs {
    const void* wpack;
    const float* scales;
    const float* norms[2 * PF_LAYERS + 1];
    const void* fast_emb;
    const float* qkv0_tbl;
    const void* tok_emb;
    const void* cb_emb;
    const float* cos_t;
    const float* sin_t;
    float eps;
    const float* xf;
    const float* slow_logits;
    int n_slow;
    float* cap;
    int cap_frames;
    float* const* hid_slot;
    float* x;
    SeqState* state;
    const SampleCfg* cfg;
    RepPenState rp;
    RngState* rng;
    uint32_t* out_codes;
    int out_cap;
    unsigned long long* edges;
    unsigned long long* prof;
    const unsigned long long* peer_stamps;
    uint32_t* ctl;
    int naps[6];
};

constexpr int PS_EDGE_CAP = 16 * 16 * 66 + 64;
constexpr size_t PS_LAYER_IMAGE = 116736;
constexpr size_t PS_HEAD_IMAGE = 16384;
constexpr size_t PS_LAYER_IMAGE_FP8 = 59392;
constexpr size_t PS_HEAD_IMAGE_FP8 = 8192;

struct SlowPersistArgs {
    const void* wpack;
    const void* hpack;
    const float* scales;
    const float* hscales;
    const float* norms;
    int n_layer, n_head_rows;
    const float* cos_t;
    const float* sin_t;
    float eps;
    float* x;
    float* logits;
    const SeqState* state;
    void* kv_pool;
    size_t layer_half;
    const int* page_table;
    int n_sl;
    unsigned long long* edges;
    unsigned long long* prof;
    const unsigned long long* peer_stamps;
    uint32_t* ctl;
    int naps[6];
    int prof_wg;
    int l2_touch;
};
constexpr int PS_STREAM_NT = 16;
size_t slow_persist_pack_bytes(int n_layer, bool fp8 = false);
size_t slow_persist_scale_floats(int n_layer);
void launch_slow_persist_pack_fp8(const LayerW* layers, int n_layer, const void* head_w, const float* head_s, int n_head_rows,
                                  const float* const* norm_ptrs, void* wpack, void* hpack, float* scales, float* norms_flat, hipStream_t st);
size_t slow_persist_edge_bytes();
void launch_slow_persist_pack(const LayerW* layers, int n_layer, const void* head_w, int n_head_rows, const float* const* norm_ptrs,
                              void* wpack, void* hpack, float* norms_flat, hipStream_t st);
void launch_slow_persist(const SlowPersistArgs& a, hipStream_t st);

bool fast_persist_supported(const ModelDims& d, int n_fast_layer, int n_cb, int cb_size);
size_t fast_persist_pack_bytes();
size_t fast_persist_edge_bytes();
void launch_fast_persist_pack(const LayerW* fast, const void* head_w, void* pack, hipStream_t st, bool fp8 = false, const float* head_s = nullptr,
                              float* scales = nullptr);
size_t fast_persist_qkv0_bytes();
void launch_fast_persist_qkv0_table(const void* pack, const float* scales, const float* norm0, const void* fast_emb, float eps, float* tbl,
                                    hipStream_t st);
void launch_fast_persist(const FastPersistArgs& a, bool sampled, hipStream_t st);
bool fast_persist_samples(float temp, int top_k, int cb_size);
void launch_pf_reduce_selftest(const float* in , float* out , hipStream_t st);

}
```

### fish-speech.rs_amd/csrc/lm_persist_slow.hip

```cpp
#include "lm_persist.h"

#include <hip/hip_runtime.h>

#include <type_traits>
#include <vector>

#include "fs_common.h"

namespace fs {

namespace {

#include "lm_persist_dev.h"
#include "lm_persist_rows_dev.h"

constexpr int PS_DROR8 = 0x128;

constexpr size_t IM_QKV4 = 0, IM_QKV1 = 8192, IM_WO = 10240, IM_W13 = 18432, IM_W2 = 83968;
static_assert(IM_W2 + 4 * 8192 == PS_LAYER_IMAGE, "image layout");
constexpr size_t I8_QKV4 = 0, I8_QKV1 = 4096, I8_WO = 6144, I8_W13 = 10240, I8_W2 = 43008;
static_assert(I8_W2 + 2 * 8192 == PS_LAYER_IMAGE_FP8, "fp8 image layout");
constexpr int PS_SC = 48, SC_QKV = 0, SC_WO = 8, SC_W13 = 12, SC_W2 = 44;

typedef float f32x2_t __attribute__((ext_vector_type(2)));
typedef __bf16 ps_bf16x8_t __attribute__((ext_vector_type(8)));
typedef float ps_f32x4_t __attribute__((ext_vector_type(4)));
static bool slow_s4_mfma() {
    static const bool v = [] { const char* e = std::getenv("FISHRT_SLOW_S4_VALU"); return !(e && std::atoi(e) != 0); }();
    return v;
}
__device__ __forceinline__ void pf_dot2x2_fp8(uint32_t w, float c0, float c1, float& acc_even, float& acc_odd) {
    const f32x2_t a = __builtin_amdgcn_cvt_pk_f32_fp8(w, false), b2 = __builtin_amdgcn_cvt_pk_f32_fp8(w, true);
    acc_even = fmaf(a.x, c0, acc_even); acc_even = fmaf(a.y, c1, acc_even);
    acc_odd = fmaf(b2.x, c0, acc_odd); acc_odd = fmaf(b2.y, c1, acc_odd);
}

constexpr int S_XS = 0;
constexpr int S_RED = S_XS + 4096;
constexpr int PS_RED = 40;
constexpr int S_QS = S_RED + 2 * 8 * PS_RED * 4;
constexpr int S_KN = S_QS + 256;
constexpr int S_VN = S_KN + 256;
constexpr int S_PART = S_VN + 256;
constexpr int S_WMAX = S_PART + 8 * 72 * 4;
constexpr int S_PAGES = S_WMAX + 64;
constexpr int S_XB = S_PAGES + 160 * 4;
constexpr int S_END = S_XB + 3 * 2048 + 8 * 16;
constexpr int PS_LDS = 96 * 1024;
static_assert(S_END <= PS_LDS, "LDS budget");

__device__ __forceinline__ void pf_sweep8u(const u64* base, const int (&unit)[8], int n, unsigned tag, u32x4 (&v)[8], bool& dead, uint32_t* ctl) {
    const u64* p[8];
#pragma unroll
    for (int i = 0; i < 8; ++i) p[i] = base + 2 * (size_t)unit[i < n ? i : 0];
    for (unsigned spins = 0;; ++spins) {
        asm volatile(
            "global_load_dwordx4 %0, %8, off sc1\n\tglobal_load_dwordx4 %1, %9, off sc1\n\tglobal_load_dwordx4 %2, %10, off sc1\n\t"
            "global_load_dwordx4 %3, %11, off sc1\n\tglobal_load_dwordx4 %4, %12, off sc1\n\tglobal_load_dwordx4 %5, %13, off sc1\n\t"
            "global_load_dwordx4 %6, %14, off sc1\n\tglobal_load_dwordx4 %7, %15, off sc1\n\ts_waitcnt vmcnt(0)"
            : "=&v"(v[0]), "=&v"(v[1]), "=&v"(v[2]), "=&v"(v[3]), "=&v"(v[4]), "=&v"(v[5]), "=&v"(v[6]), "=&v"(v[7])
            : "v"(p[0]), "v"(p[1]), "v"(p[2]), "v"(p[3]), "v"(p[4]), "v"(p[5]), "v"(p[6]), "v"(p[7])
            : "memory");
        bool ok = true;
#pragma unroll
        for (int i = 0; i < 8; ++i) ok &= pf_tags_ok(v[i], tag);
        if (ok || dead) return;
        if (spins > PF_SPIN_MAX) { dead = true; atomicAdd(ctl + 1, 1u); return; }
    }
}

template <bool NT>
__device__ __forceinline__ void ps_load16_unseen(u32x4& dst, const unsigned char* base, unsigned voff) {
    if constexpr (NT) asm volatile("global_load_dwordx4 %0, %1, %2 nt" : "=v"(dst) : "v"(voff), "s"(base));
    else asm volatile("global_load_dwordx4 %0, %1, %2" : "=v"(dst) : "v"(voff), "s"(base));
}
template <bool NT, typename V>
__device__ __forceinline__ V ps_ld_w(const V* p) {
    if constexpr (NT) return __builtin_nontemporal_load(p);
    else return *p;
}

}

__global__ __launch_bounds__(PF_THREADS) void k_ps_pack_layer(LayerW w, unsigned char* __restrict__ image , int w13_frag) {
    const int b = blockIdx.x, t = threadIdx.x;
    unsigned char* im = image + (size_t)b * PS_LAYER_IMAGE;
    const uint32_t* Wq = reinterpret_cast<const uint32_t*>(w.wqkv);
    const uint32_t* Wo = reinterpret_cast<const uint32_t*>(w.wo);
    const uint32_t* W13 = reinterpret_cast<const uint32_t*>(w.w13);
    const uint32_t* W2 = reinterpret_cast<const uint32_t*>(w.w2);
    u32x4 v;
    for (int r = 0; r < 4; ++r) v[r] = Wq[(size_t)(5 * b + r) * 512 + t];
    reinterpret_cast<u32x4*>(im + IM_QKV4)[t] = v;
    reinterpret_cast<uint32_t*>(im + IM_QKV1)[t] = Wq[(size_t)(5 * b + 4) * 512 + t];
    for (int r = 0; r < 4; ++r) v[r] = Wo[(size_t)(4 * b + r) * 512 + t];
    reinterpret_cast<u32x4*>(im + IM_WO)[t] = v;
    for (int c = 0; c < 8; ++c) {
        if (w13_frag) {
            const int rt = c >> 2, j = c & 3, wv = t >> 6, ln = t & 63;
            const size_t row = (size_t)(32 * b + 16 * rt + (ln & 15));
            for (int k = 0; k < 4; ++k) v[k] = W13[row * 512 + (size_t)(64 * wv + 16 * j + 4 * (ln >> 4) + k)];
        } else {
            for (int r = 0; r < 4; ++r) v[r] = W13[(size_t)(32 * b + 4 * c + r) * 512 + t];
        }
        reinterpret_cast<u32x4*>(im + IM_W13)[c * PF_THREADS + t] = v;
    }
    for (int q = 0; q < 4; ++q) {
        for (int r = 0; r < 4; ++r) v[r] = W2[(size_t)(4 * b + r) * 2048 + 512 * q + t];
        reinterpret_cast<u32x4*>(im + IM_W2)[q * PF_THREADS + t] = v;
    }
}
__global__ __launch_bounds__(PF_THREADS) void k_ps_pack_head(const uint32_t* __restrict__ W, int n_rows, unsigned char* __restrict__ image) {
    const int b = blockIdx.x, t = threadIdx.x;
    for (int c = 0; c < 2; ++c) {
        u32x4 v;
        for (int r = 0; r < 4; ++r) { const int row = 8 * b + 4 * c + r; v[r] = row < n_rows ? W[(size_t)row * 512 + t] : 0u; }
        reinterpret_cast<u32x4*>(image + (size_t)b * PS_HEAD_IMAGE)[c * PF_THREADS + t] = v;
    }
}
__global__ __launch_bounds__(PF_THREADS) void k_ps_pack_layer_fp8(LayerW w, unsigned char* __restrict__ image ,
                                                                  float* __restrict__ scales ) {
    const int b = blockIdx.x, t = threadIdx.x;
    unsigned char* im = image + (size_t)b * PS_LAYER_IMAGE_FP8;
    const uint16_t* Wq = reinterpret_cast<const uint16_t*>(w.wqkv);
    const uint16_t* Wo = reinterpret_cast<const uint16_t*>(w.wo);
    const uint16_t* W13 = reinterpret_cast<const uint16_t*>(w.w13);
    const uint16_t* W2 = reinterpret_cast<const uint16_t*>(w.w2);
    auto two = [](const uint16_t* W, size_t r0, size_t ld, int col) { return (uint32_t)W[r0 * ld + col] | ((uint32_t)W[(r0 + 1) * ld + col] << 16); };
    reinterpret_cast<u32x2*>(im + I8_QKV4)[t] = u32x2{two(Wq, 5 * b, 512, t), two(Wq, 5 * b + 2, 512, t)};
    reinterpret_cast<uint32_t*>(im + I8_QKV1)[t] = (uint32_t)Wq[(size_t)(5 * b + 4) * 512 + t];
    reinterpret_cast<u32x2*>(im + I8_WO)[t] = u32x2{two(Wo, 4 * b, 512, t), two(Wo, 4 * b + 2, 512, t)};
    for (int c = 0; c < 4; ++c) {
        u32x4 v;
        for (int k = 0; k < 4; ++k) v[k] = two(W13, 32 * b + 8 * c + 2 * k, 512, t);
        reinterpret_cast<u32x4*>(im + I8_W13)[c * PF_THREADS + t] = v;
    }
    for (int h = 0; h < 2; ++h) {
        u32x4 v;
        for (int qq = 0; qq < 2; ++qq) {
            const int col = 512 * (2 * h + qq) + t;
            v[2 * qq] = two(W2, 4 * b, 2048, col);
            v[2 * qq + 1] = two(W2, 4 * b + 2, 2048, col);
        }
        reinterpret_cast<u32x4*>(im + I8_W2)[h * PF_THREADS + t] = v;
    }
    if (t < PS_SC) {
        float sc = 0.f;
        if (t < 5) sc = w.s_qkv[5 * b + t];
        else if (t >= SC_WO && t < SC_WO + 4) sc = w.s_o[4 * b + t - SC_WO];
        else if (t >= SC_W13 && t < SC_W13 + 32) sc = w.s_13[32 * b + t - SC_W13];
        else if (t >= SC_W2) sc = w.s_2[4 * b + t - SC_W2];
        scales[(size_t)b * PS_SC + t] = sc;
    }
}
__global__ __launch_bounds__(PF_THREADS) void k_ps_pack_head_fp8(const uint16_t* __restrict__ W, const float* __restrict__ ws, int n_rows,
                                                                 unsigned char* __restrict__ image ,
                                                                 float* __restrict__ scales ) {
    const int b = blockIdx.x, t = threadIdx.x;
    u32x4 v;
    for (int k = 0; k < 4; ++k) {
        const int r0 = 8 * b + 2 * k;
        const uint32_t lo = r0 < n_rows ? W[(size_t)r0 * 512 + t] : 0u, hi = r0 + 1 < n_rows ? W[(size_t)(r0 + 1) * 512 + t] : 0u;
        v[k] = lo | (hi << 16);
    }
    reinterpret_cast<u32x4*>(image + (size_t)b * PS_HEAD_IMAGE_FP8)[t] = v;
    if (t < 8) scales[b * 8 + t] = 8 * b + t < n_rows ? ws[8 * b + t] : 0.f;
}
__global__ void k_ps_copy_norm(const float* __restrict__ src, float* __restrict__ dst) { dst[blockIdx.x * 256 + threadIdx.x] = src[blockIdx.x * 256 + threadIdx.x]; }

template <bool FP8, bool NT>
__global__ __launch_bounds__(PF_THREADS) void k_slow_persist(SlowPersistArgs A) {
    extern __shared__ __attribute__((aligned(16))) unsigned char smem[];
    const unsigned long long t_entry = A.prof ? wall_clock64() : 0;
    float* xs = reinterpret_cast<float*>(smem + S_XS);
    float* red = reinterpret_cast<float*>(smem + S_RED);
    float* qs = reinterpret_cast<float*>(smem + S_QS);
    float* knew = reinterpret_cast<float*>(smem + S_KN);
    float* vnew = reinterpret_cast<float*>(smem + S_VN);
    float* part = reinterpret_cast<float*>(smem + S_PART);
    float* wmax = reinterpret_cast<float*>(smem + S_WMAX);
    int* s_pages = reinterpret_cast<int*>(smem + S_PAGES);

    const int tid_k = threadIdx.x, b = blockIdx.x;
    int tid = tid_k, lane = tid & 63, wave = tid >> 6;
    const int rep = b & (PF_REPL - 1);
    u64* const edges = A.edges;
    const size_t ering = (size_t)PF_REPL * PS_EDGE_CAP;
    const u64* const my_edges = A.edges + (size_t)rep * PS_EDGE_CAP;
    auto pub = [&](unsigned e, int rr, int index, unsigned tag, float value) {
        gu64* g = (gu64*)(edges + (size_t)(e & (PF_RING - 1)) * ering + (size_t)rr * PS_EDGE_CAP + index);
        __hip_atomic_store(g, ((u64)tag << 32) | (u64)__float_as_uint(value), PF_RLX_AGENT);
    };

    if (A.state->done != 0) return;
    const int pos = A.state->pos;
    const int rpos = pos + A.state->rope_off;
    const unsigned epoch = A.ctl[0];
    const unsigned tag0 = epoch * 256u;
    const int n_sl = A.n_sl;
    const bool att = b < 16 * n_sl;
    const int ah = att ? b / n_sl : 0, as = att ? b % n_sl : 0, ag = ah >> 3;
    const int chunk_t = (pos + n_sl - 1) / n_sl;
    const int t0 = min(pos, as * chunk_t), t1 = min(pos, (as + 1) * chunk_t);
    const bool last_slice = att && as == n_sl - 1;
    const int n_tok = t1 - t0;
    const int n_tiles = att ? max((n_tok + 127) / 128, last_slice ? 1 : 0) : 0;
    if (att) {
        const int p0 = t0 >> 6;
        for (int i = tid; i < 160; i += PF_THREADS) s_pages[i] = (n_tok > 0 && p0 + i <= ((t1 - 1) >> 6)) ? A.page_table[p0 + i] : 0;
    }
    const int page_new = A.page_table[pos >> 6];
    float2 x2 = *reinterpret_cast<const float2*>(A.x + 2 * tid);
    float x0 = x2.x, x1 = x2.y;
    float rope_c = A.cos_t[(size_t)rpos * 32 + (tid & 31)], rope_s = A.sin_t[(size_t)rpos * 32 + (tid & 31)];
    __syncthreads();
    asm volatile("" : "+v"(rope_c), "+v"(rope_s));

    constexpr size_t LIMG = FP8 ? PS_LAYER_IMAGE_FP8 : PS_LAYER_IMAGE;
    const unsigned char* wimg = reinterpret_cast<const unsigned char*>(A.wpack) + (size_t)b * LIMG;
    const size_t layer_img = (size_t)PF_BLOCKS * LIMG;
    u32x4 wq4 = u32x4{0, 0, 0, 0}, wo4 = u32x4{0, 0, 0, 0}, w13[8], w2r[4];
    u32x2 wq4f = u32x2{0, 0}, wo4f = u32x2{0, 0};
    u32x4 w13f[4], w2f[2];
    uint32_t wq1;
    if constexpr (FP8) {
        wq4f = ps_ld_w<NT>(reinterpret_cast<const u32x2*>(wimg + I8_QKV4) + tid);
        wq1 = ps_ld_w<NT>(reinterpret_cast<const uint32_t*>(wimg + I8_QKV1) + tid);
    } else {
        wq4 = ps_ld_w<NT>(reinterpret_cast<const u32x4*>(wimg + IM_QKV4) + tid);
        wq1 = ps_ld_w<NT>(reinterpret_cast<const uint32_t*>(wimg + IM_QKV1) + tid);
    }
    const float* scl = FP8 ? A.scales + (size_t)b * PS_SC : nullptr;
    const size_t scl_layer = (size_t)PF_BLOCKS * PS_SC;
    u32x4 kreg[2] = {u32x4{0, 0, 0, 0}, u32x4{0, 0, 0, 0}}, vreg[2] = {u32x4{0, 0, 0, 0}, u32x4{0, 0, 0, 0}};
    bool dead = false;
    unsigned e = 0;
    int par = 0;
    const int early_mode = A.l2_touch;
    const bool s4_mfma = (early_mode & 4) != 0;
    const bool early13 = (early_mode & 1) && !att, early2 = (early_mode & 2) && !att;
    auto request_w13 = [&](const unsigned char* wl_) {
        if constexpr (FP8) {
#pragma unroll
            for (int c = 0; c < 4; ++c) ps_load16_unseen<NT>(w13f[c], wl_ + I8_W13 + (size_t)c * PF_THREADS * 16, (unsigned)tid_k * 16u);
        } else {
#pragma unroll
            for (int c = 0; c < 8; ++c) ps_load16_unseen<NT>(w13[c], wl_ + IM_W13 + (size_t)c * PF_THREADS * 16, (unsigned)tid_k * 16u);
        }
    };
    auto request_w2 = [&](const unsigned char* wl_) {
        if constexpr (FP8) {
            ps_load16_unseen<NT>(w2f[0], wl_ + I8_W2, (unsigned)tid_k * 16u); ps_load16_unseen<NT>(w2f[1], wl_ + I8_W2 + PF_THREADS * 16, (unsigned)tid_k * 16u);
        } else {
#pragma unroll
            for (int q = 0; q < 4; ++q) ps_load16_unseen<NT>(w2r[q], wl_ + IM_W2 + (size_t)q * PF_THREADS * 16, (unsigned)tid_k * 16u);
        }
    };
    unsigned long long tk[16] = {0, 0, 0, 0, 0, 0, 0, 0, 0, 0, 0, 0, 0, 0, 0, 0}, t_last = A.prof ? wall_clock64() : 0;
    const unsigned long long t_timers = t_last;
#define PS_TICK(k) do { if (A.prof) { const unsigned long long n_ = wall_clock64(); tk[k] += n_ - t_last; t_last = n_; } } while (0)

    uint32_t kv_off0[2] = {0u, 0u};
    if (att && n_tok > 0) {
#pragma unroll
        for (int u = 0; u < 2; ++u) {
            const int i = tid + PF_THREADS * u;
            const int t = min(t0 + (i >> 3), max(t1 - 1, t0));
            const int pg = s_pages[(t >> 6) - (t0 >> 6)];
            kv_off0[u] = (uint32_t)(((pg * 2 + ag) * KV_PAGE + (t & 63)) * 64 + (i & 7) * 8);
        }
    }
    auto load_kv_tile0 = [&](int l) {
        const uint16_t* kpool = reinterpret_cast<const uint16_t*>(A.kv_pool) + (size_t)l * 2 * A.layer_half;
        const uint16_t* vpool = kpool + A.layer_half;
#pragma unroll
        for (int u = 0; u < 2; ++u) {
            kreg[u] = *reinterpret_cast<const u32x4*>(kpool + kv_off0[u]);
            vreg[u] = *reinterpret_cast<const u32x4*>(vpool + kv_off0[u]);
        }
    };
    auto load_kv_tile = [&](int l, int tile) {
        const uint16_t* kpool = reinterpret_cast<const uint16_t*>(A.kv_pool) + (size_t)l * 2 * A.layer_half;
        const uint16_t* vpool = kpool + A.layer_half;
#pragma unroll
        for (int u = 0; u < 2; ++u) {
            const int i = tid + PF_THREADS * u;
            const int t = min(t0 + tile * 128 + (i >> 3), max(t1 - 1, t0));
            const int pg = s_pages[(t >> 6) - (t0 >> 6)];
            const size_t off = ((size_t)(pg * 2 + ag) * KV_PAGE + (t & 63)) * 64 + (size_t)(i & 7) * 8;
            kreg[u] = *reinterpret_cast<const u32x4*>(kpool + off);
            vreg[u] = *reinterpret_cast<const u32x4*>(vpool + off);
        }
    };

#pragma unroll 1
    for (int l = 0; l < A.n_layer; ++l) {
        const unsigned char* wl = wimg + (size_t)l * layer_img;
        {
            tid = pf_opaque(tid_k); lane = tid & 63; wave = tid >> 6;
            const float2 nw = *reinterpret_cast<const float2*>(A.norms + (size_t)(2 * l) * 1024 + 2 * tid);
            if (l > 0) {
                u32x4 v;
                pf_nap_before_sweep(A.naps[0]);
                pf_sweep1(my_edges + (size_t)(e & 3) * ering, tid, tag0 + e + 1, v, dead, A.ctl);
                x0 = __uint_as_float(v.x); x1 = __uint_as_float(v.z);
                ++e;
                PS_TICK(9);
            }
            const bool kv_late = (early_mode & 8) != 0;
            if (att && n_tok > 0 && !kv_late) load_kv_tile0(l);
            *reinterpret_cast<float2*>(xs + 2 * tid) = make_float2(x0, x1);
            const float xn0 = x0 * nw.x, xn1 = x1 * nw.y;
            float a8[8] = {0.f, 0.f, 0.f, 0.f, 0.f, 0.f, 0.f, 0.f};
            float rsc = 1.f;
            if constexpr (FP8) {
                if (tid < 64) rsc = scl[(size_t)l * scl_layer + SC_QKV + min(tid & 15, 4)];
                pf_dot2x2_fp8(wq4f.x, xn0, xn1, a8[0], a8[1]); pf_dot2x2_fp8(wq4f.y, xn0, xn1, a8[2], a8[3]);
                pf_dot2x2_fp8(wq1, xn0, xn1, a8[4], a8[6]);
                a8[6] = 0.f;
            } else {
                a8[0] = pf_dot2(wq4.x, xn0, xn1, 0.f); a8[1] = pf_dot2(wq4.y, xn0, xn1, 0.f);
                a8[2] = pf_dot2(wq4.z, xn0, xn1, 0.f); a8[3] = pf_dot2(wq4.w, xn0, xn1, 0.f);
                a8[4] = pf_dot2(wq1, xn0, xn1, 0.f);
            }
            a8[5] = fmaf(x1, x1, fmaf(x0, x0, 0.f));
            const float r8 = pf_reduce<8>(a8, lane);
            if ((lane & 7) == 0) red[(par * 8 + wave) * PS_RED + (lane >> 3)] = r8;
            __syncthreads();
            if (wave == 0) {
                const int r = min(lane & 15, 5), k = lane >> 4;
                const float* rp = red + (par * 8 + k) * PS_RED;
                float t = pf_sum_rows(rp[r] + rp[4 * PS_RED + r]);
                const float tot = pf_sum_rows(rp[5] + rp[4 * PS_RED + 5]);
                if constexpr (FP8) t *= rsc;
                if ((lane & 15) < 5) {
                    const float val = t * pf_rms_inv(tot, A.eps);
                    pub(e, k, 5 * b + r, tag0 + e + 1, val);
                    pub(e, k + 4, 5 * b + r, tag0 + e + 1, val);
                }
            }
            if (att && n_tok > 0 && kv_late) load_kv_tile0(l);
            if (early13) request_w13(wl);
            if (early2) request_w2(wl);
            par ^= 1;
            PS_TICK(1);
        }
        if constexpr (FP8) wo4f = ps_ld_w<NT>(reinterpret_cast<const u32x2*>(wl + I8_WO) + tid);
        else wo4 = ps_ld_w<NT>(reinterpret_cast<const u32x4*>(wl + IM_WO) + tid);
        if (att) {
            tid = pf_opaque(tid_k); lane = tid & 63; wave = tid >> 6;
            const u64* eb = my_edges + (size_t)(e & 3) * ering;
            if (tid < 96) {
                const int unit = tid < 32 ? 32 * ah + tid : (tid < 64 ? 512 + 32 * ag + (tid - 32) : 576 + 32 * ag + (tid - 64));
                u32x4 v;
                pf_nap_before_sweep(A.naps[1]);
                pf_sweep1(eb, unit, tag0 + e + 1, v, dead, A.ctl);
                const float a0 = __uint_as_float(v.x), a1 = __uint_as_float(v.z);
                const int j = tid & 31;
                const float c = rope_c, s = rope_s;
                if (tid < 32) {
                    *reinterpret_cast<float2*>(qs + 2 * j) = make_float2((a0 * c - a1 * s) * 0.125f, (a0 * s + a1 * c) * 0.125f);
                } else if (tid < 64) {
                    const uint32_t k0 = f32_to_bf16_rne(a0 * c - a1 * s), k1 = f32_to_bf16_rne(a0 * s + a1 * c);
                    *reinterpret_cast<float2*>(knew + 2 * j) = make_float2(bf_lo(k0), bf_lo(k1));
                    if (last_slice && (ah & 7) == 0)
                        reinterpret_cast<uint32_t*>(reinterpret_cast<uint16_t*>(A.kv_pool) + (size_t)l * 2 * A.layer_half +
                                                    ((size_t)(page_new * 2 + ag) * KV_PAGE + (pos & 63)) * 64)[j] = k0 | (k1 << 16);
                } else {
                    const uint32_t v0 = f32_to_bf16_rne(a0), v1 = f32_to_bf16_rne(a1);
                    *reinterpret_cast<float2*>(vnew + 2 * j) = make_float2(bf_lo(v0), bf_lo(v1));
                    if (last_slice && (ah & 7) == 0)
                        reinterpret_cast<uint32_t*>(reinterpret_cast<uint16_t*>(A.kv_pool) + (size_t)l * 2 * A.layer_half + A.layer_half +
                                                    ((size_t)(page_new * 2 + ag) * KV_PAGE + (pos & 63)) * 64)[j] = v0 | (v1 << 16);
                }
            }
            ++e;
            __syncthreads();
            PS_TICK(10);
            float run_m = -1e30f, run_l = 0.f, ro[8] = {0.f, 0.f, 0.f, 0.f, 0.f, 0.f, 0.f, 0.f};
            const int du = tid & 7;
            float qv[8];
            {
                const float4 q0 = *reinterpret_cast<const float4*>(qs + du * 8), q1 = *reinterpret_cast<const float4*>(qs + du * 8 + 4);
                qv[0] = q0.x; qv[1] = q0.y; qv[2] = q0.z; qv[3] = q0.w; qv[4] = q1.x; qv[5] = q1.y; qv[6] = q1.z; qv[7] = q1.w;
            }
            for (int tile = 0; tile < n_tiles; ++tile) {
                if (tile > 0) load_kv_tile(l, tile);
                float sc[3];
                bool valid[3];
#pragma unroll
                for (int u = 0; u < 2; ++u) {
                    const int t = t0 + tile * 128 + ((tid + PF_THREADS * u) >> 3);
                    valid[u] = t < t1;
                    const u32x4 kk = kreg[u];
                    float a = 0.f;
                    a = fmaf(qv[0], bf_lo(kk.x), a); a = fmaf(qv[1], bf_hi(kk.x), a); a = fmaf(qv[2], bf_lo(kk.y), a); a = fmaf(qv[3], bf_hi(kk.y), a);
                    a = fmaf(qv[4], bf_lo(kk.z), a); a = fmaf(qv[5], bf_hi(kk.z), a); a = fmaf(qv[6], bf_lo(kk.w), a); a = fmaf(qv[7], bf_hi(kk.w), a);
                    a += pf_dpp<PF_XOR1>(a); a += pf_dpp<PF_XOR2>(a); a += pf_dpp<PF_HALF_MIRROR>(a);
                    sc[u] = valid[u] ? a : -1e30f;
                }
                const bool has_new = last_slice && tile == n_tiles - 1 && tid < 8;
                {
                    float a = 0.f;
#pragma unroll
                    for (int i = 0; i < 8; ++i) a = fmaf(qv[i], knew[du * 8 + i], a);
                    a += pf_dpp<PF_XOR1>(a); a += pf_dpp<PF_XOR2>(a); a += pf_dpp<PF_HALF_MIRROR>(a);
                    valid[2] = has_new;
                    sc[2] = has_new ? a : -1e30f;
                }
                float m = fmaxf(fmaxf(sc[0], sc[1]), sc[2]);
                m = fmaxf(m, pf_dpp<PF_XOR1>(m)); m = fmaxf(m, pf_dpp<PF_XOR2>(m)); m = fmaxf(m, pf_dpp<PF_HALF_MIRROR>(m)); m = fmaxf(m, pf_dpp<PF_MIRROR>(m));
                m = fmaxf(fmaxf(__int_as_float(__builtin_amdgcn_readlane(__float_as_int(m), 15)), __int_as_float(__builtin_amdgcn_readlane(__float_as_int(m), 31))),
                          fmaxf(__int_as_float(__builtin_amdgcn_readlane(__float_as_int(m), 47)), __int_as_float(__builtin_amdgcn_readlane(__float_as_int(m), 63))));
                const float mn = fmaxf(run_m, m), ca = __expf(run_m - mn);
                run_l *= ca;
#pragma unroll
                for (int i = 0; i < 8; ++i) ro[i] *= ca;
#pragma unroll
                for (int u = 0; u < 3; ++u) {
                    const float p = valid[u] ? __expf(sc[u] - mn) : 0.f;
                    if (du == 0) run_l += p;
                    if (u < 2) {
                        const u32x4 vv = vreg[u];
                        ro[0] = fmaf(p, bf_lo(vv.x), ro[0]); ro[1] = fmaf(p, bf_hi(vv.x), ro[1]); ro[2] = fmaf(p, bf_lo(vv.y), ro[2]); ro[3] = fmaf(p, bf_hi(vv.y), ro[3]);
                        ro[4] = fmaf(p, bf_lo(vv.z), ro[4]); ro[5] = fmaf(p, bf_hi(vv.z), ro[5]); ro[6] = fmaf(p, bf_lo(vv.w), ro[6]); ro[7] = fmaf(p, bf_hi(vv.w), ro[7]);
                    } else {
#pragma unroll
                        for (int i = 0; i < 8; ++i) ro[i] = fmaf(p, vnew[du * 8 + i], ro[i]);
                    }
                }
                run_m = mn;
            }
            {
                float o9[9];
#pragma unroll
                for (int i = 0; i < 8; ++i) o9[i] = ro[i];
                o9[8] = run_l;
#pragma unroll
                for (int i = 0; i < 9; ++i) {
                    float t = o9[i];
                    t += pf_dpp<PS_DROR8>(t);
                    const auto r = __builtin_amdgcn_permlane16_swap(__float_as_uint(t), __float_as_uint(t), false, false);
                    t = __uint_as_float(r[0]) + __uint_as_float(r[1]);
                    const auto r2 = __builtin_amdgcn_permlane32_swap(__float_as_uint(t), __float_as_uint(t), false, false);
                    o9[i] = __uint_as_float(r2[0]) + __uint_as_float(r2[1]);
                }
                if (lane < 8) {
#pragma unroll
                    for (int i = 0; i < 8; ++i) part[wave * 72 + lane * 8 + i] = o9[i];
                    if (lane == 0) { part[wave * 72 + 64] = o9[8]; wmax[wave] = run_m; }
                }
            }
            __syncthreads();
            if (tid < 66) {
                float M = wmax[0];
#pragma unroll
                for (int w = 1; w < 8; ++w) M = fmaxf(M, wmax[w]);
                float val = 0.f;
                if (tid == 64) val = M;
                else {
#pragma unroll
                    for (int w = 0; w < 8; ++w) val = fmaf(part[w * 72 + (tid < 64 ? tid : 64)], __expf(wmax[w] - M), val);
                }
                const int base = (ah * n_sl + as) * 66;
#pragma unroll
                for (int rr = 0; rr < PF_REPL; ++rr) pub(e, rr, base + tid, tag0 + e + 1, val);
            }
            __syncthreads();
            PS_TICK(2);
        } else {
            ++e;
        }
        {
            tid = pf_opaque(tid_k); lane = tid & 63; wave = tid >> 6;
            const int h = tid >> 5, j = tid & 31;
            const u64* eb = my_edges + (size_t)(e & 3) * ering;
            float rsc = 1.f;
            if constexpr (FP8) { if (tid < 64) rsc = scl[(size_t)l * scl_layer + SC_WO + min(tid & 15, 3)]; }
            float mn = -1e30f, L = 0.f, at0 = 0.f, at1 = 0.f;
            float sm[16], sl_[16], so0[16], so1[16];
            pf_nap_before_sweep(A.naps[2]);
            if (n_sl > 4) {
                const unsigned off_o = (unsigned)((h * n_sl * 66 + 2 * j) * 8), off_ml = (unsigned)((h * n_sl * 66 + 64) * 8);
#pragma unroll
                for (int rd = 0; rd < 2; ++rd) {
                    if (8 * rd < n_sl) {
                        const u64* sb[8];
                        u32x4 vo[8], vm[8];
#pragma unroll
                        for (int k = 0; k < 8; ++k) sb[k] = eb + (size_t)(8 * rd + k) * 66;
                        pr_sweep_att8(sb, off_o, off_ml, tag0 + e + 1, vo, vm, dead, A.ctl);
#pragma unroll
                        for (int k = 0; k < 8; ++k) {
                            so0[8 * rd + k] = __uint_as_float(vo[k].x); so1[8 * rd + k] = __uint_as_float(vo[k].z);
                            sm[8 * rd + k] = __uint_as_float(vm[k].x); sl_[8 * rd + k] = __uint_as_float(vm[k].z);
                        }
                    } else {
#pragma unroll
                        for (int k = 0; k < 8; ++k) { so0[8 * rd + k] = 0.f; so1[8 * rd + k] = 0.f; sm[8 * rd + k] = -1e30f; sl_[8 * rd + k] = 0.f; }
                    }
                }
            } else
#pragma unroll
            for (int g4 = 0; g4 < 4; ++g4) {
                const int s0 = 4 * g4;
                if (s0 < n_sl) {
                    int unit[8];
                    u32x4 v[8];
                    const int ns = min(4, n_sl - s0);
#pragma unroll
                    for (int k = 0; k < 4; ++k) {
                        const int gbase = (h * n_sl + s0 + (k < ns ? k : 0)) * 66;
                        unit[2 * k] = (gbase + 2 * j) >> 1;
                        unit[2 * k + 1] = (gbase + 64) >> 1;
                    }
                    pf_sweep8u(eb, unit, 2 * ns, tag0 + e + 1, v, dead, A.ctl);
#pragma unroll
                    for (int k = 0; k < 4; ++k) {
                        so0[s0 + k] = __uint_as_float(v[2 * k].x); so1[s0 + k] = __uint_as_float(v[2 * k].z);
                        sm[s0 + k] = __uint_as_float(v[2 * k + 1].x); sl_[s0 + k] = __uint_as_float(v[2 * k + 1].z);
                    }
                } else {
#pragma unroll
                    for (int k = 0; k < 4; ++k) { so0[s0 + k] = 0.f; so1[s0 + k] = 0.f; sm[s0 + k] = -1e30f; sl_[s0 + k] = 0.f; }
                }
            }
            ++e;
            PS_TICK(11);
            if constexpr (FP8) {
                asm volatile("" : "+v"(rsc));
                asm volatile("" : "+v"(wo4f));
                if (!early13) request_w13(wl);
            } else {
                asm volatile("" : "+v"(wo4));
                if (!early13) request_w13(wl);
            }
            auto merge = [&](auto NC) {
                constexpr int NS = decltype(NC)::value;
#pragma unroll
                for (int s = 0; s < NS; ++s) mn = fmaxf(mn, sm[s]);
                float ex[NS];
#pragma unroll
                for (int s = 0; s < NS; ++s) { ex[s] = __expf(sm[s] - mn); L += sl_[s] * ex[s]; }
                const float inv = 1.f / L;
#pragma unroll
                for (int s = 0; s < NS; ++s) {
                    const float wj = ex[s] * inv;
                    at0 = fmaf(wj, so0[s], at0);
                    at1 = fmaf(wj, so1[s], at1);
                }
            };
            switch (n_sl) {
                case 1: merge(std::integral_constant<int, 1>{}); break;
                case 2: merge(std::integral_constant<int, 2>{}); break;
                case 4: merge(std::integral_constant<int, 4>{}); break;
                case 8: merge(std::integral_constant<int, 8>{}); break;
                default: merge(std::integral_constant<int, 16>{}); break;
            }
            float a4[4] = {0.f, 0.f, 0.f, 0.f};
            if constexpr (FP8) {
                pf_dot2x2_fp8(wo4f.x, at0, at1, a4[0], a4[1]); pf_dot2x2_fp8(wo4f.y, at0, at1, a4[2], a4[3]);
            } else {
                a4[0] = pf_dot2(wo4.x, at0, at1, 0.f); a4[1] = pf_dot2(wo4.y, at0, at1, 0.f);
                a4[2] = pf_dot2(wo4.z, at0, at1, 0.f); a4[3] = pf_dot2(wo4.w, at0, at1, 0.f);
            }
            const float r4 = pf_reduce<4>(a4, lane);
            if ((lane & 15) == 0) red[(par * 8 + wave) * PS_RED + (lane >> 4)] = r4;
            float xres = 0.f;
            if (tid < 64) xres = xs[4 * b + min(tid & 15, 3)];
            __syncthreads();
            if (wave == 0) {
                const int r = min(lane & 15, 3), k = lane >> 4;
                const float* rp = red + (par * 8 + k) * PS_RED;
                float t = pf_sum_rows(rp[r] + rp[4 * PS_RED + r]);
                if constexpr (FP8) t *= rsc;
                if ((lane & 15) < 4) {
                    pub(e, k, 4 * b + r, tag0 + e + 1, xres + t);
                    pub(e, k + 4, 4 * b + r, tag0 + e + 1, xres + t);
                }
            }
            par ^= 1;
            PS_TICK(3);
        }
        {
            tid = pf_opaque(tid_k); lane = tid & 63; wave = tid >> 6;
            const float2 nw = *reinterpret_cast<const float2*>(A.norms + (size_t)(2 * l + 1) * 1024 + 2 * tid);
            float rsa = 1.f, rsb = 1.f;
            if constexpr (FP8) {
                if (tid < 64) { rsa = scl[(size_t)l * scl_layer + SC_W13 + 2 * (tid & 15)]; rsb = scl[(size_t)l * scl_layer + SC_W13 + 2 * (tid & 15) + 1]; }
            }
            u32x4 v;
            pf_nap_before_sweep(A.naps[3]);
            pf_sweep1(my_edges + (size_t)(e & 3) * ering, tid, tag0 + e + 1, v, dead, A.ctl);
            ++e;
            PS_TICK(12);
            float nwx = nw.x, nwy = nw.y;
            asm volatile("" : "+v"(nwx), "+v"(nwy));
            if constexpr (FP8) asm volatile("" : "+v"(rsa), "+v"(rsb));
            if constexpr (FP8) {
#pragma unroll
                for (int c = 0; c < 4; ++c) asm volatile("" : "+v"(w13f[c]));
            } else {
#pragma unroll
                for (int c = 0; c < 8; ++c) asm volatile("" : "+v"(w13[c]));
            }
            if (!early2) request_w2(wl);
            x0 = __uint_as_float(v.x); x1 = __uint_as_float(v.z);
            *reinterpret_cast<float2*>(xs + 2 * tid) = make_float2(x0, x1);
            const float xn0 = x0 * nwx, xn1 = x1 * nwy;
            const float ssw = pf_wave_sum(fmaf(x1, x1, fmaf(x0, x0, 0.f)));
            if (lane == 0) red[(par * 8 + wave) * PS_RED + 32] = ssw;
            if (!FP8 && s4_mfma) {
                uint32_t* xb = reinterpret_cast<uint32_t*>(smem + S_XB);
                uint32_t pk[3];
                {
                    const uint32_t h0 = __float_as_uint(xn0) & 0xFFFF0000u, h1 = __float_as_uint(xn1) & 0xFFFF0000u;
                    const float r0 = xn0 - __uint_as_float(h0), r1 = xn1 - __uint_as_float(h1);
                    const uint32_t m0 = __float_as_uint(r0) & 0xFFFF0000u, m1 = __float_as_uint(r1) & 0xFFFF0000u;
                    const uint32_t l0 = __float_as_uint(r0 - __uint_as_float(m0)), l1 = __float_as_uint(r1 - __uint_as_float(m1));
                    pk[0] = (h0 >> 16) | h1; pk[1] = (m0 >> 16) | m1; pk[2] = (l0 >> 16) | (l1 & 0xFFFF0000u);
                }
                xb[tid] = pk[0]; xb[512 + tid] = pk[1]; xb[1024 + tid] = pk[2];
                if (lane < 4) xb[1536 + 4 * wave + lane] = 0u;
                __builtin_amdgcn_wave_barrier();
                const int n = lane & 15, q4 = lane >> 4;
                const u32x4* xbv = reinterpret_cast<const u32x4*>(smem + S_XB);
                const int zslot = 384 + wave;
                const int src = n < 3 ? n * 128 + 16 * wave + q4 : zslot;
                ps_f32x4_t acc0 = {0.f, 0.f, 0.f, 0.f}, acc1 = {0.f, 0.f, 0.f, 0.f};
#pragma unroll
                for (int j = 0; j < 4; ++j) {
                    const ps_bf16x8_t bv = __builtin_bit_cast(ps_bf16x8_t, xbv[n < 3 ? src + 4 * j : zslot]);
                    acc0 = __builtin_amdgcn_mfma_f32_16x16x32_bf16(__builtin_bit_cast(ps_bf16x8_t, w13[j]), bv, acc0, 0, 0, 0);
                    acc1 = __builtin_amdgcn_mfma_f32_16x16x32_bf16(__builtin_bit_cast(ps_bf16x8_t, w13[4 + j]), bv, acc1, 0, 0, 0);
                }
#pragma unroll
                for (int r = 0; r < 4; ++r) {
                    acc0[r] += pf_dpp<0x101>(acc0[r]) + pf_dpp<0x102>(acc0[r]);
                    acc1[r] += pf_dpp<0x101>(acc1[r]) + pf_dpp<0x102>(acc1[r]);
                }
                if (n == 0) {
                    *reinterpret_cast<float4*>(red + (par * 8 + wave) * PS_RED + 4 * q4) = make_float4(acc0[0], acc0[1], acc0[2], acc0[3]);
                    *reinterpret_cast<float4*>(red + (par * 8 + wave) * PS_RED + 16 + 4 * q4) = make_float4(acc1[0], acc1[1], acc1[2], acc1[3]);
                }
            } else {
#pragma unroll
                for (int half = 0; half < 2; ++half) {
                    float a16[16] = {0.f, 0.f, 0.f, 0.f, 0.f, 0.f, 0.f, 0.f, 0.f, 0.f, 0.f, 0.f, 0.f, 0.f, 0.f, 0.f};
                    if constexpr (FP8) {
    #pragma unroll
                        for (int c = 0; c < 2; ++c) {
                            const u32x4 w = w13f[half * 2 + c];
                            pf_dot2x2_fp8(w.x, xn0, xn1, a16[8 * c], a16[8 * c + 1]); pf_dot2x2_fp8(w.y, xn0, xn1, a16[8 * c + 2], a16[8 * c + 3]);
                            pf_dot2x2_fp8(w.z, xn0, xn1, a16[8 * c + 4], a16[8 * c + 5]); pf_dot2x2_fp8(w.w, xn0, xn1, a16[8 * c + 6], a16[8 * c + 7]);
                        }
                    } else {
    #pragma unroll
                        for (int c = 0; c < 4; ++c) {
                            const u32x4 w = w13[half * 4 + c];
                            a16[4 * c] = pf_dot2(w.x, xn0, xn1, 0.f); a16[4 * c + 1] = pf_dot2(w.y, xn0, xn1, 0.f);
                            a16[4 * c + 2] = pf_dot2(w.z, xn0, xn1, 0.f); a16[4 * c + 3] = pf_dot2(w.w, xn0, xn1, 0.f);
                        }
                    }
                    const float r16 = pf_reduce<16>(a16, lane);
                    if ((lane & 3) == 0) red[(par * 8 + wave) * PS_RED + half * 16 + (lane >> 2)] = r16;
                }
            }
            __syncthreads();
            if (wave == 0) {
                const int jj = lane & 15, k = lane >> 4;
                const float* rp = red + (par * 8 + k) * PS_RED;
                const float2 g2 = *reinterpret_cast<const float2*>(rp + 2 * jj), h2 = *reinterpret_cast<const float2*>(rp + 4 * PS_RED + 2 * jj);
                float ga = pf_sum_rows(g2.x + h2.x), gb = pf_sum_rows(g2.y + h2.y);
                const float tot = pf_sum_rows(rp[32] + rp[4 * PS_RED + 32]);
                const float dni = pf_rms_inv(tot, A.eps);
                if constexpr (FP8) { ga *= rsa; gb *= rsb; }
                ga *= dni; gb *= dni;
                const float act = pf_silu(ga) * gb;
                pub(e, k, 16 * b + jj, tag0 + e + 1, act);
                pub(e, k + 4, 16 * b + jj, tag0 + e + 1, act);
            }
            par ^= 1;
            PS_TICK(4);
        }
        {
            tid = pf_opaque(tid_k); lane = tid & 63; wave = tid >> 6;
            u32x4 v[4];
            pf_nap_before_sweep(A.naps[4]);
            pf_sweep4(my_edges + (size_t)(e & 3) * ering, tid, tag0 + e + 1, v, dead, A.ctl);
            ++e;
            PS_TICK(13);
            if constexpr (FP8) { asm volatile("" : "+v"(w2f[0]), "+v"(w2f[1])); }
            else {
#pragma unroll
                for (int q = 0; q < 4; ++q) asm volatile("" : "+v"(w2r[q]));
            }
            float rsc = 1.f;
            if constexpr (FP8) { if (tid < 64) rsc = scl[(size_t)l * scl_layer + SC_W2 + min(tid & 15, 3)]; }
            if (l + 1 < A.n_layer) {
                if constexpr (FP8) {
                    wq4f = ps_ld_w<NT>(reinterpret_cast<const u32x2*>(wl + layer_img + I8_QKV4) + tid);
                    wq1 = ps_ld_w<NT>(reinterpret_cast<const uint32_t*>(wl + layer_img + I8_QKV1) + tid);
                } else {
                    wq4 = ps_ld_w<NT>(reinterpret_cast<const u32x4*>(wl + layer_img + IM_QKV4) + tid);
                    wq1 = ps_ld_w<NT>(reinterpret_cast<const uint32_t*>(wl + layer_img + IM_QKV1) + tid);
                }
            }
            float a4[4] = {0.f, 0.f, 0.f, 0.f};
            if constexpr (FP8) {
#pragma unroll
                for (int q = 0; q < 4; ++q) {
                    const u32x4 w = w2f[q >> 1];
                    const float c0 = __uint_as_float(v[q].x), c1 = __uint_as_float(v[q].z);
                    pf_dot2x2_fp8((q & 1) ? w.z : w.x, c0, c1, a4[0], a4[1]); pf_dot2x2_fp8((q & 1) ? w.w : w.y, c0, c1, a4[2], a4[3]);
                }
            } else {
#pragma unroll
            for (int q = 0; q < 4; ++q) {
                const u32x4 w = w2r[q];
                const float c0 = __uint_as_float(v[q].x), c1 = __uint_as_float(v[q].z);
                a4[0] = pf_dot2(w.x, c0, c1, a4[0]); a4[1] = pf_dot2(w.y, c0, c1, a4[1]);
                a4[2] = pf_dot2(w.z, c0, c1, a4[2]); a4[3] = pf_dot2(w.w, c0, c1, a4[3]);
            }
            }
            const float r4 = pf_reduce<4>(a4, lane);
            if ((lane & 15) == 0) red[(par * 8 + wave) * PS_RED + (lane >> 4)] = r4;
            float xres = 0.f;
            if (tid < 64) xres = xs[4 * b + min(tid & 15, 3)];
            __syncthreads();
            if (wave == 0) {
                const int r = min(lane & 15, 3), k = lane >> 4;
                const float* rp = red + (par * 8 + k) * PS_RED;
                float t = pf_sum_rows(rp[r] + rp[4 * PS_RED + r]);
                if constexpr (FP8) t *= rsc;
                if ((lane & 15) < 4) {
                    pub(e, k, 4 * b + r, tag0 + e + 1, xres + t);
                    pub(e, k + 4, 4 * b + r, tag0 + e + 1, xres + t);
                }
            }
            par ^= 1;
            PS_TICK(5);
        }
    }
    {
        tid = pf_opaque(tid_k); lane = tid & 63; wave = tid >> 6;
        const float2 nw = *reinterpret_cast<const float2*>(A.norms + (size_t)(2 * A.n_layer) * 1024 + 2 * tid);
        const u32x4* hp = reinterpret_cast<const u32x4*>(reinterpret_cast<const unsigned char*>(A.hpack) + (size_t)b * (FP8 ? PS_HEAD_IMAGE_FP8 : PS_HEAD_IMAGE));
        const u32x4 h0 = ps_ld_w<NT>(hp + tid), h1 = FP8 ? u32x4{0, 0, 0, 0} : ps_ld_w<NT>(hp + PF_THREADS + tid);
        float rsc = 1.f;
        if constexpr (FP8) { if (tid < 64) rsc = A.hscales[8 * b + min(tid & 15, 7)]; }
        u32x4 v;
        pf_nap_before_sweep(A.naps[5]);
        pf_sweep1(my_edges + (size_t)(e & 3) * ering, tid, tag0 + e + 1, v, dead, A.ctl);
        ++e;
        PS_TICK(14);
        x0 = __uint_as_float(v.x); x1 = __uint_as_float(v.z);
        if (b == 0) *reinterpret_cast<float2*>(A.x + 2 * tid) = make_float2(x0, x1);
        const float xn0 = x0 * nw.x, xn1 = x1 * nw.y;
        float a8[8] = {0.f, 0.f, 0.f, 0.f, 0.f, 0.f, 0.f, 0.f};
        if constexpr (FP8) {
            pf_dot2x2_fp8(h0.x, xn0, xn1, a8[0], a8[1]); pf_dot2x2_fp8(h0.y, xn0, xn1, a8[2], a8[3]);
            pf_dot2x2_fp8(h0.z, xn0, xn1, a8[4], a8[5]); pf_dot2x2_fp8(h0.w, xn0, xn1, a8[6], a8[7]);
        } else {
            a8[0] = pf_dot2(h0.x, xn0, xn1, 0.f); a8[1] = pf_dot2(h0.y, xn0, xn1, 0.f); a8[2] = pf_dot2(h0.z, xn0, xn1, 0.f); a8[3] = pf_dot2(h0.w, xn0, xn1, 0.f);
            a8[4] = pf_dot2(h1.x, xn0, xn1, 0.f); a8[5] = pf_dot2(h1.y, xn0, xn1, 0.f); a8[6] = pf_dot2(h1.z, xn0, xn1, 0.f); a8[7] = pf_dot2(h1.w, xn0, xn1, 0.f);
        }
        const float ssw = pf_wave_sum(fmaf(x1, x1, fmaf(x0, x0, 0.f)));
        const float r8 = pf_reduce<8>(a8, lane);
        if ((lane & 7) == 0) red[(par * 8 + wave) * PS_RED + (lane >> 3)] = r8;
        if (lane == 0) red[(par * 8 + wave) * PS_RED + 8] = ssw;
        __syncthreads();
        if (wave == 0) {
            const int r = min(lane & 15, 7), k = lane >> 4;
            const float* rp = red + (par * 8 + k) * PS_RED;
            float t = pf_sum_rows(rp[r] + rp[4 * PS_RED + r]);
            const float tot = pf_sum_rows(rp[8] + rp[4 * PS_RED + 8]);
            if constexpr (FP8) t *= rsc;
            if (lane < 8 && 8 * b + r < A.n_head_rows) A.logits[8 * b + r] = t * pf_rms_inv(tot, A.eps);
        }
        PS_TICK(6);
    }
    if (b == 0 && tid == 0) A.ctl[0] = epoch + 1;
    if (A.prof && b == A.prof_wg && tid == 0) {
        for (int k = 0; k < 16; ++k) A.prof[k] += tk[k];
        const unsigned long long t_end = wall_clock64(), peer_end = A.peer_stamps ? A.peer_stamps[0] : 0;
        if (peer_end && t_entry > peer_end && t_entry - peer_end < 20000) { A.prof[17] += t_entry - peer_end; A.prof[20] += 1; }
        A.prof[18] += t_timers - t_entry;
        A.prof[19] += t_end - t_last;
        A.prof[16] = t_end;
    }
#undef PS_TICK
}

size_t slow_persist_pack_bytes(int n_layer, bool fp8) { return (size_t)n_layer * PF_BLOCKS * (fp8 ? PS_LAYER_IMAGE_FP8 : PS_LAYER_IMAGE); }
size_t slow_persist_scale_floats(int n_layer) { return (size_t)n_layer * PF_BLOCKS * PS_SC + (size_t)PF_BLOCKS * 8; }
size_t slow_persist_edge_bytes() { return (size_t)PF_RING * PF_REPL * PS_EDGE_CAP * 8; }

void launch_slow_persist_pack(const LayerW* layers, int n_layer, const void* head_w, int n_head_rows, const float* const* norm_ptrs,
                              void* wpack, void* hpack, float* norms_flat, hipStream_t st) {
    for (int l = 0; l < n_layer; ++l)
        hipLaunchKernelGGL(k_ps_pack_layer, dim3(PF_BLOCKS), dim3(PF_THREADS), 0, st, layers[l],
                           reinterpret_cast<unsigned char*>(wpack) + (size_t)l * PF_BLOCKS * PS_LAYER_IMAGE, slow_s4_mfma() ? 1 : 0);
    hipLaunchKernelGGL(k_ps_pack_head, dim3(PF_BLOCKS), dim3(PF_THREADS), 0, st, reinterpret_cast<const uint32_t*>(head_w), n_head_rows,
                       reinterpret_cast<unsigned char*>(hpack));
    for (int i = 0; i < 2 * n_layer + 1; ++i)
        hipLaunchKernelGGL(k_ps_copy_norm, dim3(4), dim3(256), 0, st, norm_ptrs[i], norms_flat + (size_t)i * 1024);
    FS_HIP(hipGetLastError());
}

void launch_slow_persist_pack_fp8(const LayerW* layers, int n_layer, const void* head_w, const float* head_s, int n_head_rows,
                                  const float* const* norm_ptrs, void* wpack, void* hpack, float* scales, float* norms_flat, hipStream_t st) {
    for (int l = 0; l < n_layer; ++l)
        hipLaunchKernelGGL(k_ps_pack_layer_fp8, dim3(PF_BLOCKS), dim3(PF_THREADS), 0, st, layers[l],
                           reinterpret_cast<unsigned char*>(wpack) + (size_t)l * PF_BLOCKS * PS_LAYER_IMAGE_FP8, scales + (size_t)l * PF_BLOCKS * PS_SC);
    hipLaunchKernelGGL(k_ps_pack_head_fp8, dim3(PF_BLOCKS), dim3(PF_THREADS), 0, st, reinterpret_cast<const uint16_t*>(head_w), head_s, n_head_rows,
                       reinterpret_cast<unsigned char*>(hpack), scales + (size_t)n_layer * PF_BLOCKS * PS_SC);
    for (int i = 0; i < 2 * n_layer + 1; ++i)
        hipLaunchKernelGGL(k_ps_copy_norm, dim3(4), dim3(256), 0, st, norm_ptrs[i], norms_flat + (size_t)i * 1024);
    FS_HIP(hipGetLastError());
}

void launch_slow_persist(const SlowPersistArgs& a, hipStream_t st) {
    using kern_t = void (*)(SlowPersistArgs);
    static const kern_t kern[2][2] = {{k_slow_persist<false, false>, k_slow_persist<false, true>}, {k_slow_persist<true, false>, k_slow_persist<true, true>}};
    static bool attr_set = false;
    if (!attr_set) {
        for (int i = 0; i < 4; ++i)
            FS_HIP(hipFuncSetAttribute(reinterpret_cast<const void*>(kern[i >> 1][i & 1]), hipFuncAttributeMaxDynamicSharedMemorySize, PS_LDS));
        attr_set = true;
    }
    SlowPersistArgs b2 = a;
    if (!a.scales && slow_s4_mfma()) b2.l2_touch |= 4;
    const bool nt = (a.l2_touch & PS_STREAM_NT) != 0;
    hipLaunchKernelGGL(kern[a.scales ? 1 : 0][nt ? 1 : 0], dim3(PF_BLOCKS), dim3(PF_THREADS), PS_LDS, st, b2);
    FS_HIP(hipGetLastError());
}

}
```

Baseline: 1913.

## Fold Q projection into attention blocks of the slow persistent kernel

Adds a q-fold variant of the slow persistent transformer kernel for bf16 weights. Each attention block computes its own head's Q projection from a repacked Q weight image held in LDS. Dedicated workgroups compute the K/V rows and write them to the KV cache, and the new token's score is merged in the output-combine stage. This removes one grid-wide edge exchange per layer (four edges per block instead of five) in exchange for more LDS, an extra packed weight image, and extra per-layer weight prefetches through global_load_lds.

```diff
diff --git a/fish-speech.rs_amd/csrc/lm_engine.hip b/fish-speech.rs_amd/csrc/lm_engine.hip
--- a/fish-speech.rs_amd/csrc/lm_engine.hip
+++ b/fish-speech.rs_amd/csrc/lm_engine.hip
@@ -1899,6 +1899,9 @@
         if (use_pslow_) {
             FS_HIP(hipMemcpy(pr, d_sctl_.as<uint32_t>() + 16, sizeof(pr), hipMemcpyDeviceToHost));
             FS_HIP(hipMemset(d_sctl_.as<uint32_t>() + 16, 0, sizeof(pr)));
+            const SlowPersistArgs pa = pslow_args();
+            fprintf(stderr, slow_persist_runs_qfold(pa) ? "slow persist path: q-fold, four edges per block (S1 = x sweep + k/v rows, S2 = q product + tiles), n_sl %d\n"
+                                                        : "slow persist path: five stages per block, n_sl %d\n", pa.n_sl);
             fprintf(stderr, "slow persist prof (us/frame, workgroup %d; wait+work): S1 %.1f+%.1f  S2 %.1f+%.1f  S3 %.1f+%.1f  S4 %.1f+%.1f  S5 %.1f+%.1f  head %.1f+%.1f\n",
                     getenv("FISHRT_PERSIST_PROF_WG") ? atoi(getenv("FISHRT_PERSIST_PROF_WG")) : 0, pr[9] * f, pr[1] * f, pr[10] * f, pr[2] * f, pr[11] * f, pr[3] * f,
                     pr[12] * f, pr[4] * f, pr[13] * f, pr[5] * f, pr[14] * f, pr[6] * f);
@@ -2396,6 +2399,7 @@
     static constexpr int kNapsFast[6] = {16, 16, 16, 16, 16, 16}, kNapsSlow[6] = {20, 16, 6, 36, 36, 12};
     static constexpr int kNapsFastSampled[6] = {12, 16, 12, 20, 12, 16}, kNapsSlowFp8[6] = {20, 4, 28, 24, 24, 0};
     static constexpr bool kSlowStreamNt = true, kSlowStreamNtFp8 = true;
+    static constexpr bool kSlowQfold = true;
     static void set_naps(int (&naps)[6], const char* env, const int (&dflt)[6]) {
         for (int i = 0; i < 6; ++i) naps[i] = dflt[i];
         if (const char* v = getenv(env)) {
@@ -2448,6 +2452,11 @@
             if (FP8) launch_slow_persist_pack_fp8(slow_.data(), a_.n_layer, slow_head_w(), slow_head_s(), n_audio_, np.data(), d_spack_.p, d_hpack_.p,
                                                   d_sscl_.as<float>(), d_snorms_.as<float>(), st_);
             else launch_slow_persist_pack(slow_.data(), a_.n_layer, slow_head_w(), n_audio_, np.data(), d_spack_.p, d_hpack_.p, d_snorms_.as<float>(), st_);
+            slow_qfold_ = !FP8 && (getenv("FISHRT_SLOW_QFOLD") ? atoi(getenv("FISHRT_SLOW_QFOLD")) != 0 : kSlowQfold);
+            if (slow_qfold_) {
+                if (!d_sqpack_.p) d_sqpack_.alloc(slow_persist_qf_bytes(a_.n_layer));
+                launch_slow_persist_pack_qf(slow_.data(), a_.n_layer, d_sqpack_.p, st_);
+            }
             FS_HIP(hipStreamSynchronize(st_));
             pslow_ok_ = true;
         }
@@ -2476,6 +2485,7 @@
         bool stream_nt = kFp8 ? kSlowStreamNtFp8 : kSlowStreamNt;
         if (const char* c = getenv("FISHRT_SLOW_STREAM")) stream_nt = strcmp(c, "nt") == 0;
         if (stream_nt) A.l2_touch |= PS_STREAM_NT;
+        A.qpack = slow_qfold_ ? d_sqpack_.p : nullptr;
         return A;
     }
     bool fold_slow_sampler() const { return use_persist_ && n_audio_ <= 2048; }
@@ -2770,6 +2780,8 @@
     hipEvent_t ev_pf_ = nullptr;
     PrefillLane join_{st_pf_};
     DevBuf d_spack_, d_hpack_, d_snorms_, d_sedges_, d_sctl_;
+    DevBuf d_sqpack_;
+    bool slow_qfold_ = false;
     PrefillLane main_{st_};
     DevBuf d_bprompt_;
     DevBuf d_xfrows_, d_lrows_, d_lfast_, d_fast_state_, d_fast_table_, d_rwords_;
diff --git a/fish-speech.rs_amd/csrc/lm_persist.h b/fish-speech.rs_amd/csrc/lm_persist.h
--- a/fish-speech.rs_amd/csrc/lm_persist.h
+++ b/fish-speech.rs_amd/csrc/lm_persist.h
@@ -56,6 +56,13 @@
 constexpr size_t PS_HEAD_IMAGE = 16384;
 constexpr size_t PS_LAYER_IMAGE_FP8 = 59392;
 constexpr size_t PS_HEAD_IMAGE_FP8 = 8192;
+constexpr size_t PS_QF_HEAD = 64 * 1024 * 2;
+constexpr size_t PS_QF_KV = 16 * PS_QF_HEAD;
+constexpr size_t PS_QF_KV_WG = 4096;
+constexpr size_t PS_QF_LAYER_IMAGE = PS_QF_KV + 128 * PS_QF_KV_WG;
+constexpr int PS_QF_QOFF = 16 * 8 * 66;
+constexpr int PS_QF_KVOFF = PS_QF_QOFF + 1024;
+static_assert(PS_QF_KVOFF + 256 <= PS_EDGE_CAP, "q-fold attention edge");
 
 struct SlowPersistArgs {
     const void* wpack;
@@ -81,10 +88,14 @@
     int naps[6];
     int prof_wg;
     int l2_touch;
+    const void* qpack;
 };
 constexpr int PS_STREAM_NT = 16;
 size_t slow_persist_pack_bytes(int n_layer, bool fp8 = false);
 size_t slow_persist_scale_floats(int n_layer);
+size_t slow_persist_qf_bytes(int n_layer);
+void launch_slow_persist_pack_qf(const LayerW* layers, int n_layer, void* qpack, hipStream_t st);
+bool slow_persist_runs_qfold(const SlowPersistArgs& a);
 void launch_slow_persist_pack_fp8(const LayerW* layers, int n_layer, const void* head_w, const float* head_s, int n_head_rows,
                                   const float* const* norm_ptrs, void* wpack, void* hpack, float* scales, float* norms_flat, hipStream_t st);
 size_t slow_persist_edge_bytes();
diff --git a/fish-speech.rs_amd/csrc/lm_persist_slow.hip b/fish-speech.rs_amd/csrc/lm_persist_slow.hip
--- a/fish-speech.rs_amd/csrc/lm_persist_slow.hip
+++ b/fish-speech.rs_amd/csrc/lm_persist_slow.hip
@@ -48,6 +48,11 @@
 constexpr int S_END = S_XB + 3 * 2048 + 8 * 16;
 constexpr int PS_LDS = 96 * 1024;
 static_assert(S_END <= PS_LDS, "LDS budget");
+constexpr int S_QP = (S_END + 15) & ~15;
+constexpr int S_WQ = (S_QP + 8 * 64 * 4 + 1023) & ~1023;
+constexpr int PS_LDS_QF = S_WQ + (int)PS_QF_HEAD;
+static_assert(PS_LDS_QF <= 160 * 1024, "LDS budget of the q-fold instantiations");
+static_assert(PS_QF_HEAD == 8 * 16 * 1024, "8 waves x 16 fragment chunks");
 
 __device__ __forceinline__ void pf_sweep8u(const u64* base, const int (&unit)[8], int n, unsigned tag, u32x4 (&v)[8], bool& dead, uint32_t* ctl) {
     const u64* p[8];
@@ -79,6 +84,47 @@
     if constexpr (NT) return __builtin_nontemporal_load(p);
     else return *p;
 }
+
+__device__ __forceinline__ void ps_glds16(const unsigned char* gsrc, unsigned lds_dst) {
+    unsigned keep;
+    asm volatile("s_mov_b32 %0, m0\n\ts_mov_b32 m0, %2\n\ts_nop 0\n\tglobal_load_lds_dwordx4 %1, off\n\ts_mov_b32 m0, %0"
+                 : "=&s"(keep) : "v"(gsrc), "s"(lds_dst) : "memory");
+}
+
+#define PS_QF_SL(k, off) "global_load_dwordx4 %[o" #k "], %[oo], %[eb] offset:" #off " sc1\n\tglobal_load_dwordx4 %[m" #k "], %[om], %[eb] offset:" #off " sc1\n\t"
+#define PS_QF_TAIL "global_load_dwordx4 %[q], %[oq], %[eb] sc1\n\tglobal_load_dwordx4 %[k], %[ok], %[eb] sc1\n\tglobal_load_dwordx4 %[v], %[ok], %[eb] offset:1024 sc1\n\ts_waitcnt vmcnt(0)"
+#define PS_QF_OUT2(k) [o##k] "=&v"(vo[k]), [m##k] "=&v"(vm[k])
+#define PS_QF_INS : [oo] "v"(off_o), [om] "v"(off_ml), [oq] "v"(off_q), [ok] "v"(off_k), [eb] "s"(eb) : "memory"
+template <int NS>
+__device__ __forceinline__ void ps_sweep_qf(const u64* eb, unsigned off_o, unsigned off_ml, unsigned off_q, unsigned off_k, unsigned tag,
+                                            u32x4 (&vo)[8], u32x4 (&vm)[8], u32x4& vq, u32x4& vk, u32x4& vv, bool& dead, uint32_t* ctl) {
+    static_assert(NS == 1 || NS == 2 || NS == 4 || NS == 8, "slice counts of the q-fold path");
+    static_assert(7 * 528 < 4096 && 66 * 8 == 528, "slice stride as a 13-bit instruction offset");
+    for (unsigned spins = 0;; ++spins) {
+        if constexpr (NS == 1)
+            asm volatile(PS_QF_SL(0, 0) PS_QF_TAIL
+                         : PS_QF_OUT2(0), [q] "=&v"(vq), [k] "=&v"(vk), [v] "=&v"(vv) PS_QF_INS);
+        else if constexpr (NS == 2)
+            asm volatile(PS_QF_SL(0, 0) PS_QF_SL(1, 528) PS_QF_TAIL
+                         : PS_QF_OUT2(0), PS_QF_OUT2(1), [q] "=&v"(vq), [k] "=&v"(vk), [v] "=&v"(vv) PS_QF_INS);
+        else if constexpr (NS == 4)
+            asm volatile(PS_QF_SL(0, 0) PS_QF_SL(1, 528) PS_QF_SL(2, 1056) PS_QF_SL(3, 1584) PS_QF_TAIL
+                         : PS_QF_OUT2(0), PS_QF_OUT2(1), PS_QF_OUT2(2), PS_QF_OUT2(3), [q] "=&v"(vq), [k] "=&v"(vk), [v] "=&v"(vv) PS_QF_INS);
+        else
+            asm volatile(PS_QF_SL(0, 0) PS_QF_SL(1, 528) PS_QF_SL(2, 1056) PS_QF_SL(3, 1584) PS_QF_SL(4, 2112) PS_QF_SL(5, 2640) PS_QF_SL(6, 3168) PS_QF_SL(7, 3696) PS_QF_TAIL
+                         : PS_QF_OUT2(0), PS_QF_OUT2(1), PS_QF_OUT2(2), PS_QF_OUT2(3), PS_QF_OUT2(4), PS_QF_OUT2(5), PS_QF_OUT2(6), PS_QF_OUT2(7),
+                           [q] "=&v"(vq), [k] "=&v"(vk), [v] "=&v"(vv) PS_QF_INS);
+        bool ok = pf_tags_ok(vq, tag) && pf_tags_ok(vk, tag) && pf_tags_ok(vv, tag);
+#pragma unroll
+        for (int i = 0; i < NS; ++i) ok &= pf_tags_ok(vo[i], tag) && pf_tags_ok(vm[i], tag);
+        if (ok || dead) return;
+        if (spins > PF_SPIN_MAX) { dead = true; atomicAdd(ctl + 1, 1u); return; }
+    }
+}
+#undef PS_QF_SL
+#undef PS_QF_TAIL
+#undef PS_QF_OUT2
+#undef PS_QF_INS
 
 }
 
@@ -110,6 +156,23 @@
         reinterpret_cast<u32x4*>(im + IM_W2)[q * PF_THREADS + t] = v;
     }
 }
+__global__ __launch_bounds__(PF_THREADS) void k_ps_pack_qf(LayerW w, unsigned char* __restrict__ qimg ) {
+    const int b = blockIdx.x, t = threadIdx.x;
+    const uint32_t* Wq = reinterpret_cast<const uint32_t*>(w.wqkv);
+    if (b < 16) {
+        const int wv = t >> 6, ln = t & 63;
+        for (int c = 0; c < 16; ++c) {
+            const int rt = c >> 2, j = c & 3;
+            const size_t row = (size_t)(64 * b + 16 * rt + (ln & 15));
+            u32x4 v;
+            for (int k = 0; k < 4; ++k) v[k] = Wq[row * 512 + (size_t)(64 * wv + 16 * j + 4 * (ln >> 4) + k)];
+            reinterpret_cast<u32x4*>(qimg + (size_t)b * PS_QF_HEAD)[(16 * wv + c) * 64 + ln] = v;
+        }
+    } else {
+        const size_t r0 = 1024 + 2 * (size_t)(b - 16);
+        reinterpret_cast<u32x2*>(qimg + PS_QF_KV + (size_t)(b - 16) * PS_QF_KV_WG)[t] = u32x2{Wq[r0 * 512 + t], Wq[(r0 + 1) * 512 + t]};
+    }
+}
 __global__ __launch_bounds__(PF_THREADS) void k_ps_pack_head(const uint32_t* __restrict__ W, int n_rows, unsigned char* __restrict__ image) {
     const int b = blockIdx.x, t = threadIdx.x;
     for (int c = 0; c < 2; ++c) {
@@ -168,8 +231,9 @@
 }
 __global__ void k_ps_copy_norm(const float* __restrict__ src, float* __restrict__ dst) { dst[blockIdx.x * 256 + threadIdx.x] = src[blockIdx.x * 256 + threadIdx.x]; }
 
-template <bool FP8, bool NT>
+template <bool FP8, bool NT, bool QF = false>
 __global__ __launch_bounds__(PF_THREADS) void k_slow_persist(SlowPersistArgs A) {
+    static_assert(!(QF && FP8), "the q-fold path has bf16 images only");
     extern __shared__ __attribute__((aligned(16))) unsigned char smem[];
     const unsigned long long t_entry = A.prof ? wall_clock64() : 0;
     float* xs = reinterpret_cast<float*>(smem + S_XS);
@@ -199,10 +263,12 @@
     const unsigned tag0 = epoch * 256u;
     const int n_sl = A.n_sl;
     const bool att = b < 16 * n_sl;
-    const int ah = att ? b / n_sl : 0, as = att ? b % n_sl : 0, ag = ah >> 3;
+    const int ah = att ? (QF ? (b & 7) + 8 * ((b >> 3) / n_sl) : b / n_sl) : 0, as = att ? (QF ? (b >> 3) % n_sl : b % n_sl) : 0, ag = ah >> 3;
     const int chunk_t = (pos + n_sl - 1) / n_sl;
     const int t0 = min(pos, as * chunk_t), t1 = min(pos, (as + 1) * chunk_t);
-    const bool last_slice = att && as == n_sl - 1;
+    const bool last_slice = !QF && att && as == n_sl - 1;
+    const bool kvw = QF && b >= 128;
+    const int kvi = b - 128;
     const int n_tok = t1 - t0;
     const int n_tiles = att ? max((n_tok + 127) / 128, last_slice ? 1 : 0) : 0;
     if (att) {
@@ -213,6 +279,9 @@
     float2 x2 = *reinterpret_cast<const float2*>(A.x + 2 * tid);
     float x0 = x2.x, x1 = x2.y;
     float rope_c = A.cos_t[(size_t)rpos * 32 + (tid & 31)], rope_s = A.sin_t[(size_t)rpos * 32 + (tid & 31)];
+    if constexpr (QF) {
+        if (kvw) { rope_c = A.cos_t[(size_t)rpos * 32 + (kvi & 31)]; rope_s = A.sin_t[(size_t)rpos * 32 + (kvi & 31)]; }
+    }
     __syncthreads();
     asm volatile("" : "+v"(rope_c), "+v"(rope_s));
 
@@ -223,7 +292,22 @@
     u32x2 wq4f = u32x2{0, 0}, wo4f = u32x2{0, 0};
     u32x4 w13f[4], w2f[2];
     uint32_t wq1;
-    if constexpr (FP8) {
+    const unsigned char* const qimg = reinterpret_cast<const unsigned char*>(A.qpack);
+    u32x2 wkv = u32x2{0, 0};
+    const int wave_u = __builtin_amdgcn_readfirstlane(tid_k >> 6);
+    const unsigned lds_wq = (unsigned)(uintptr_t)(__attribute__((address_space(3))) unsigned char*)(smem + S_WQ) + (unsigned)wave_u * 16384u;
+    auto request_wq = [&](int l_, auto C0, auto C1) {
+        const unsigned char* src = qimg + (size_t)l_ * PS_QF_LAYER_IMAGE + (size_t)ah * PS_QF_HEAD + (size_t)wave_u * 16384 + (size_t)(tid_k & 63) * 16;
+#pragma unroll
+        for (int c = decltype(C0)::value; c < decltype(C1)::value; ++c) ps_glds16(src + c * 1024, __builtin_amdgcn_readfirstlane(lds_wq + c * 1024));
+    };
+    using qf_c0 = std::integral_constant<int, 0>;
+    using qf_c8 = std::integral_constant<int, 8>;
+    using qf_c16 = std::integral_constant<int, 16>;
+    if constexpr (QF) {
+        if (att) request_wq(0, qf_c0{}, qf_c16{});
+        if (kvw) wkv = ps_ld_w<NT>(reinterpret_cast<const u32x2*>(qimg + PS_QF_KV + (size_t)kvi * PS_QF_KV_WG) + tid);
+    } else if constexpr (FP8) {
         wq4f = ps_ld_w<NT>(reinterpret_cast<const u32x2*>(wimg + I8_QKV4) + tid);
         wq1 = ps_ld_w<NT>(reinterpret_cast<const uint32_t*>(wimg + I8_QKV1) + tid);
     } else {
@@ -293,9 +377,65 @@
         }
     };
 
+    if constexpr (QF) { if (att && n_tok > 0) load_kv_tile0(0); }
 #pragma unroll 1
     for (int l = 0; l < A.n_layer; ++l) {
         const unsigned char* wl = wimg + (size_t)l * layer_img;
+        float qf_xn0 = 0.f, qf_xn1 = 0.f;
+        if constexpr (QF) {
+            tid = pf_opaque(tid_k); lane = tid & 63; wave = tid >> 6;
+            const float2 nw = *reinterpret_cast<const float2*>(A.norms + (size_t)(2 * l) * 1024 + 2 * tid);
+            if (l > 0) {
+                u32x4 v;
+                pf_nap_before_sweep(A.naps[0]);
+                pf_sweep1(my_edges + (size_t)(e & 3) * ering, tid, tag0 + e + 1, v, dead, A.ctl);
+                x0 = __uint_as_float(v.x); x1 = __uint_as_float(v.z);
+                ++e;
+            } else if (att) {
+                asm volatile("s_waitcnt vmcnt(0)" ::: "memory");
+            }
+            PS_TICK(9);
+            float nwx = nw.x, nwy = nw.y;
+            asm volatile("" : "+v"(nwx), "+v"(nwy));
+            if (att) {
+#pragma unroll
+                for (int u = 0; u < 2; ++u) asm volatile("" : "+v"(kreg[u]), "+v"(vreg[u]));
+            }
+            if (kvw) asm volatile("" : "+v"(wkv));
+            *reinterpret_cast<float2*>(xs + 2 * tid) = make_float2(x0, x1);
+            qf_xn0 = x0 * nwx; qf_xn1 = x1 * nwy;
+            if (kvw) {
+                float a4[4] = {pf_dot2(wkv.x, qf_xn0, qf_xn1, 0.f), pf_dot2(wkv.y, qf_xn0, qf_xn1, 0.f), fmaf(x1, x1, fmaf(x0, x0, 0.f)), 0.f};
+                const float r4 = pf_reduce<4>(a4, lane);
+                if ((lane & 15) == 0) red[(par * 8 + wave) * PS_RED + (lane >> 4)] = r4;
+                __syncthreads();
+                if (wave == 0) {
+                    const int k = lane >> 4, r = lane & 15;
+                    const float* rp = red + (par * 8 + k) * PS_RED;
+                    const float a0 = pf_sum_rows(rp[0] + rp[4 * PS_RED]), a1 = pf_sum_rows(rp[1] + rp[4 * PS_RED + 1]);
+                    const float rinv = pf_rms_inv(pf_sum_rows(rp[2] + rp[4 * PS_RED + 2]), A.eps);
+                    const float y0 = a0 * rinv, y1 = a1 * rinv;
+                    const bool is_k = kvi < 64;
+                    const uint32_t u0 = f32_to_bf16_rne(is_k ? y0 * rope_c - y1 * rope_s : y0), u1 = f32_to_bf16_rne(is_k ? y0 * rope_s + y1 * rope_c : y1);
+                    if (r < 2) {
+                        const float val = bf_lo(r == 0 ? u0 : u1);
+                        pub(e, k, PS_QF_KVOFF + 2 * kvi + r, tag0 + e + 1, val);
+                        pub(e, k + 4, PS_QF_KVOFF + 2 * kvi + r, tag0 + e + 1, val);
+                    }
+                    if (lane == 0) {
+                        const int ri = kvi & 63, g = ri >> 5, j = ri & 31;
+                        reinterpret_cast<uint32_t*>(reinterpret_cast<uint16_t*>(A.kv_pool) + (size_t)l * 2 * A.layer_half + (is_k ? 0 : A.layer_half) +
+                                                    ((size_t)(page_new * 2 + g) * KV_PAGE + (pos & 63)) * 64)[j] = u0 | (u1 << 16);
+                    }
+                }
+            } else if (!att) {
+                __syncthreads();
+            }
+            if (early13) request_w13(wl);
+            if (early2) request_w2(wl);
+            par ^= 1;
+            PS_TICK(1);
+        } else
         {
             tid = pf_opaque(tid_k); lane = tid & 63; wave = tid >> 6;
             const float2 nw = *reinterpret_cast<const float2*>(A.norms + (size_t)(2 * l) * 1024 + 2 * tid);
@@ -349,6 +489,61 @@
         else wo4 = ps_ld_w<NT>(reinterpret_cast<const u32x4*>(wl + IM_WO) + tid);
         if (att) {
             tid = pf_opaque(tid_k); lane = tid & 63; wave = tid >> 6;
+            if constexpr (QF) {
+                uint32_t* xb = reinterpret_cast<uint32_t*>(smem + S_XB);
+                float* qp = reinterpret_cast<float*>(smem + S_QP);
+                {
+                    const uint32_t h0 = __float_as_uint(qf_xn0) & 0xFFFF0000u, h1 = __float_as_uint(qf_xn1) & 0xFFFF0000u;
+                    const float r0 = qf_xn0 - __uint_as_float(h0), r1 = qf_xn1 - __uint_as_float(h1);
+                    const uint32_t m0 = __float_as_uint(r0) & 0xFFFF0000u, m1 = __float_as_uint(r1) & 0xFFFF0000u;
+                    const uint32_t l0 = __float_as_uint(r0 - __uint_as_float(m0)), l1 = __float_as_uint(r1 - __uint_as_float(m1));
+                    xb[tid] = (h0 >> 16) | h1; xb[512 + tid] = (m0 >> 16) | m1; xb[1024 + tid] = (l0 >> 16) | (l1 & 0xFFFF0000u);
+                }
+                if (lane < 4) xb[1536 + 4 * wave + lane] = 0u;
+                const float ssw = pf_wave_sum(fmaf(x1, x1, fmaf(x0, x0, 0.f)));
+                if (lane == 0) red[(par * 8 + wave) * PS_RED + 32] = ssw;
+                __builtin_amdgcn_wave_barrier();
+                const int n = lane & 15, q4 = lane >> 4;
+                const u32x4* xbv = reinterpret_cast<const u32x4*>(smem + S_XB);
+                const u32x4* wqv = reinterpret_cast<const u32x4*>(smem + S_WQ) + (size_t)wave * 1024 + lane;
+                const int zslot = 384 + wave;
+                const int src = n < 3 ? n * 128 + 16 * wave + q4 : zslot;
+                ps_bf16x8_t bv[4];
+#pragma unroll
+                for (int j = 0; j < 4; ++j) bv[j] = __builtin_bit_cast(ps_bf16x8_t, xbv[n < 3 ? src + 4 * j : zslot]);
+#pragma unroll
+                for (int rt = 0; rt < 4; ++rt) {
+                    ps_f32x4_t acc = {0.f, 0.f, 0.f, 0.f};
+#pragma unroll
+                    for (int j = 0; j < 4; ++j)
+                        acc = __builtin_amdgcn_mfma_f32_16x16x32_bf16(__builtin_bit_cast(ps_bf16x8_t, wqv[(4 * rt + j) * 64]), bv[j], acc, 0, 0, 0);
+#pragma unroll
+                    for (int r = 0; r < 4; ++r) acc[r] += pf_dpp<0x101>(acc[r]) + pf_dpp<0x102>(acc[r]);
+                    if (n == 0) *reinterpret_cast<float4*>(qp + wave * 64 + 16 * rt + 4 * q4) = make_float4(acc[0], acc[1], acc[2], acc[3]);
+                }
+                __syncthreads();
+                if (tid < 32) {
+                    float a0 = 0.f, a1 = 0.f, tot = 0.f;
+#pragma unroll
+                    for (int w = 0; w < 8; ++w) {
+                        const float2 p2 = *reinterpret_cast<const float2*>(qp + w * 64 + 2 * tid);
+                        a0 += p2.x; a1 += p2.y; tot += red[(par * 8 + w) * PS_RED + 32];
+                    }
+                    const float rinv = pf_rms_inv(tot, A.eps);
+                    a0 *= rinv; a1 *= rinv;
+                    const float c = rope_c, s = rope_s;
+                    const float q0 = (a0 * c - a1 * s) * 0.125f, q1 = (a0 * s + a1 * c) * 0.125f;
+                    *reinterpret_cast<float2*>(qs + 2 * tid) = make_float2(q0, q1);
+                    if (as == 0) {
+#pragma unroll
+                        for (int rr = 0; rr < PF_REPL; ++rr) {
+                            pub(e, rr, PS_QF_QOFF + 64 * ah + 2 * tid, tag0 + e + 1, q0);
+                            pub(e, rr, PS_QF_QOFF + 64 * ah + 2 * tid + 1, tag0 + e + 1, q1);
+                        }
+                    }
+                }
+                par ^= 1;
+            } else {
             const u64* eb = my_edges + (size_t)(e & 3) * ering;
             if (tid < 96) {
                 const int unit = tid < 32 ? 32 * ah + tid : (tid < 64 ? 512 + 32 * ag + (tid - 32) : 576 + 32 * ag + (tid - 64));
@@ -375,6 +570,7 @@
                 }
             }
             ++e;
+            }
             __syncthreads();
             PS_TICK(10);
             float run_m = -1e30f, run_l = 0.f, ro[8] = {0.f, 0.f, 0.f, 0.f, 0.f, 0.f, 0.f, 0.f};
@@ -400,7 +596,8 @@
                     sc[u] = valid[u] ? a : -1e30f;
                 }
                 const bool has_new = last_slice && tile == n_tiles - 1 && tid < 8;
-                {
+                if constexpr (QF) { valid[2] = false; sc[2] = -1e30f; }
+                else {
                     float a = 0.f;
 #pragma unroll
                     for (int i = 0; i < 8; ++i) a = fmaf(qv[i], knew[du * 8 + i], a);
@@ -417,7 +614,7 @@
 #pragma unroll
                 for (int i = 0; i < 8; ++i) ro[i] *= ca;
 #pragma unroll
-                for (int u = 0; u < 3; ++u) {
+                for (int u = 0; u < (QF ? 2 : 3); ++u) {
                     const float p = valid[u] ? __expf(sc[u] - mn) : 0.f;
                     if (du == 0) run_l += p;
                     if (u < 2) {
@@ -467,9 +664,12 @@
                 for (int rr = 0; rr < PF_REPL; ++rr) pub(e, rr, base + tid, tag0 + e + 1, val);
             }
             __syncthreads();
+            if constexpr (QF) {
+                if (l + 1 < A.n_layer) request_wq(l + 1, qf_c0{}, qf_c8{});
+            }
             PS_TICK(2);
         } else {
-            ++e;
+            if constexpr (!QF) ++e;
         }
         {
             tid = pf_opaque(tid_k); lane = tid & 63; wave = tid >> 6;
@@ -480,6 +680,31 @@
             float mn = -1e30f, L = 0.f, at0 = 0.f, at1 = 0.f;
             float sm[16], sl_[16], so0[16], so1[16];
             pf_nap_before_sweep(A.naps[2]);
+            if constexpr (QF) {
+                const unsigned off_o = (unsigned)((h * n_sl * 66 + 2 * j) * 8), off_ml = (unsigned)((h * n_sl * 66 + 64) * 8);
+                const unsigned off_q = (unsigned)((PS_QF_QOFF + 64 * h + 2 * j) * 8), off_k = (unsigned)((PS_QF_KVOFF + 64 * (h >> 3) + 2 * j) * 8);
+                auto sweep_qf = [&](auto NC) {
+                    constexpr int NS = decltype(NC)::value;
+                    u32x4 vo[8], vm[8], vq, vk, vv;
+                    ps_sweep_qf<NS>(eb, off_o, off_ml, off_q, off_k, tag0 + e + 1, vo, vm, vq, vk, vv, dead, A.ctl);
+#pragma unroll
+                    for (int k = 0; k < 16; ++k) {
+                        if (k < NS) {
+                            so0[k] = __uint_as_float(vo[k].x); so1[k] = __uint_as_float(vo[k].z);
+                            sm[k] = __uint_as_float(vm[k].x); sl_[k] = __uint_as_float(vm[k].z);
+                        } else if (k > NS) { so0[k] = 0.f; so1[k] = 0.f; sm[k] = -1e30f; sl_[k] = 0.f; }
+                    }
+                    const float part_s = fmaf(__uint_as_float(vq.x), __uint_as_float(vk.x), __uint_as_float(vq.z) * __uint_as_float(vk.z));
+                    sm[NS] = pf_allsum32(part_s); sl_[NS] = 1.f;
+                    so0[NS] = __uint_as_float(vv.x); so1[NS] = __uint_as_float(vv.z);
+                };
+                switch (n_sl) {
+                    case 1: sweep_qf(std::integral_constant<int, 1>{}); break;
+                    case 2: sweep_qf(std::integral_constant<int, 2>{}); break;
+                    case 4: sweep_qf(std::integral_constant<int, 4>{}); break;
+                    default: sweep_qf(std::integral_constant<int, 8>{}); break;
+                }
+            } else
             if (n_sl > 4) {
                 const unsigned off_o = (unsigned)((h * n_sl * 66 + 2 * j) * 8), off_ml = (unsigned)((h * n_sl * 66 + 64) * 8);
 #pragma unroll
@@ -550,6 +775,14 @@
                     at1 = fmaf(wj, so1[s], at1);
                 }
             };
+            if constexpr (QF) {
+                switch (n_sl) {
+                    case 1: merge(std::integral_constant<int, 2>{}); break;
+                    case 2: merge(std::integral_constant<int, 3>{}); break;
+                    case 4: merge(std::integral_constant<int, 5>{}); break;
+                    default: merge(std::integral_constant<int, 9>{}); break;
+                }
+            } else
             switch (n_sl) {
                 case 1: merge(std::integral_constant<int, 1>{}); break;
                 case 2: merge(std::integral_constant<int, 2>{}); break;
@@ -680,6 +913,9 @@
                 pub(e, k, 16 * b + jj, tag0 + e + 1, act);
                 pub(e, k + 4, 16 * b + jj, tag0 + e + 1, act);
             }
+            if constexpr (QF) {
+                if (att && l + 1 < A.n_layer) { __syncthreads(); request_wq(l + 1, qf_c8{}, qf_c16{}); }
+            }
             par ^= 1;
             PS_TICK(4);
         }
@@ -698,7 +934,9 @@
             float rsc = 1.f;
             if constexpr (FP8) { if (tid < 64) rsc = scl[(size_t)l * scl_layer + SC_W2 + min(tid & 15, 3)]; }
             if (l + 1 < A.n_layer) {
-                if constexpr (FP8) {
+                if constexpr (QF) {
+                    if (kvw) wkv = ps_ld_w<NT>(reinterpret_cast<const u32x2*>(qimg + (size_t)(l + 1) * PS_QF_LAYER_IMAGE + PS_QF_KV + (size_t)kvi * PS_QF_KV_WG) + tid);
+                } else if constexpr (FP8) {
                     wq4f = ps_ld_w<NT>(reinterpret_cast<const u32x2*>(wl + layer_img + I8_QKV4) + tid);
                     wq1 = ps_ld_w<NT>(reinterpret_cast<const uint32_t*>(wl + layer_img + I8_QKV1) + tid);
                 } else {
@@ -737,6 +975,9 @@
                     pub(e, k, 4 * b + r, tag0 + e + 1, xres + t);
                     pub(e, k + 4, 4 * b + r, tag0 + e + 1, xres + t);
                 }
+            }
+            if constexpr (QF) {
+                if (att && n_tok > 0 && l + 1 < A.n_layer) load_kv_tile0(l + 1);
             }
             par ^= 1;
             PS_TICK(5);
@@ -820,19 +1061,31 @@
     FS_HIP(hipGetLastError());
 }
 
+size_t slow_persist_qf_bytes(int n_layer) { return (size_t)n_layer * PS_QF_LAYER_IMAGE; }
+void launch_slow_persist_pack_qf(const LayerW* layers, int n_layer, void* qpack, hipStream_t st) {
+    for (int l = 0; l < n_layer; ++l)
+        hipLaunchKernelGGL(k_ps_pack_qf, dim3(16 + 128), dim3(PF_THREADS), 0, st, layers[l], reinterpret_cast<unsigned char*>(qpack) + (size_t)l * PS_QF_LAYER_IMAGE);
+    FS_HIP(hipGetLastError());
+}
+bool slow_persist_runs_qfold(const SlowPersistArgs& a) { return a.qpack && !a.scales && a.n_sl <= 8; }
+
 void launch_slow_persist(const SlowPersistArgs& a, hipStream_t st) {
     using kern_t = void (*)(SlowPersistArgs);
     static const kern_t kern[2][2] = {{k_slow_persist<false, false>, k_slow_persist<false, true>}, {k_slow_persist<true, false>, k_slow_persist<true, true>}};
+    static const kern_t kern_qf[2] = {k_slow_persist<false, false, true>, k_slow_persist<false, true, true>};
     static bool attr_set = false;
     if (!attr_set) {
         for (int i = 0; i < 4; ++i)
             FS_HIP(hipFuncSetAttribute(reinterpret_cast<const void*>(kern[i >> 1][i & 1]), hipFuncAttributeMaxDynamicSharedMemorySize, PS_LDS));
+        for (int i = 0; i < 2; ++i)
+            FS_HIP(hipFuncSetAttribute(reinterpret_cast<const void*>(kern_qf[i]), hipFuncAttributeMaxDynamicSharedMemorySize, PS_LDS_QF));
         attr_set = true;
     }
     SlowPersistArgs b2 = a;
     if (!a.scales && slow_s4_mfma()) b2.l2_touch |= 4;
     const bool nt = (a.l2_touch & PS_STREAM_NT) != 0;
-    hipLaunchKernelGGL(kern[a.scales ? 1 : 0][nt ? 1 : 0], dim3(PF_BLOCKS), dim3(PF_THREADS), PS_LDS, st, b2);
+    if (slow_persist_runs_qfold(a)) hipLaunchKernelGGL(kern_qf[nt ? 1 : 0], dim3(PF_BLOCKS), dim3(PF_THREADS), PS_LDS_QF, st, b2);
+    else hipLaunchKernelGGL(kern[a.scales ? 1 : 0][nt ? 1 : 0], dim3(PF_BLOCKS), dim3(PF_THREADS), PS_LDS, st, b2);
     FS_HIP(hipGetLastError());
 }
 
```

Result: slower. 1792 (-6.3%).
